# mimbres/neural-audio-fp

Hardware: NVIDIA B200
Metric: search_queries_per_s (higher is better)
Workload: dtype bf16 scan, f32 re-rank

## Files before the change

include/nafp.h:

```cpp
#ifndef NAFP_H_
#define NAFP_H_

#include <stdint.h>

#ifdef __cplusplus
extern "C" {
#endif

typedef struct nafp_ctx nafp_ctx;
typedef struct nafp_index nafp_index;

typedef enum {
    NAFP_OK = 0,
    NAFP_ERR_INVALID = -1,
    NAFP_ERR_CUDA = -2,
    NAFP_ERR_STATE = -3,
    NAFP_ERR_UNSUPPORTED = -4
} nafp_status;

enum { NAFP_INDEX_FLAT_L2 = 0, NAFP_INDEX_IVFPQ = 1, NAFP_INDEX_IVF_FLAT = 2, NAFP_INDEX_IVFPQR = 3 };

int nafp_version(void);
const char* nafp_last_error(void);
int nafp_device_count(void);

int nafp_ctx_create(int device, nafp_ctx** out);
int nafp_ctx_destroy(nafp_ctx* ctx);
int nafp_sync(nafp_ctx* ctx);
void* nafp_ctx_stream(nafp_ctx* ctx);
int nafp_ctx_set_stream(nafp_ctx* ctx, void* cuda_stream);
int64_t nafp_ctx_launch_count(nafp_ctx* ctx);

int nafp_malloc(nafp_ctx* ctx, int64_t bytes, void** out_dev);
int nafp_free(nafp_ctx* ctx, void* dev);
int nafp_malloc_host(nafp_ctx* ctx, int64_t bytes, void** out_host);
int nafp_free_host(nafp_ctx* ctx, void* host);
int nafp_memcpy_h2d(nafp_ctx* ctx, void* dst_dev, const void* src_host, int64_t bytes);
int nafp_memcpy_d2h(nafp_ctx* ctx, void* dst_host, const void* src_dev, int64_t bytes);
int nafp_timer_start(nafp_ctx* ctx);
int nafp_timer_stop(nafp_ctx* ctx, float* out_ms);

int nafp_synth_fp_rows(nafp_ctx* ctx, int64_t seed, int64_t row0, int64_t n_rows, int32_t track_len,
                       float rho, float* out_dev);
int nafp_synth_audio(nafp_ctx* ctx, int64_t seed, int64_t seg0, int64_t n_seg, float* out_dev);


int nafp_weights_load(nafp_ctx* ctx, const float* const* conv_w, const float* const* conv_b,
                      const float* const* ln_g, const float* const* ln_b, const float* div_w1,
                      const float* div_b1, const float* div_w2, const float* div_b2);

int nafp_logmel_forward(nafp_ctx* ctx, const float* x_dev, int64_t n_seg, int64_t group_size,
                        float* mel_dev);

int nafp_logmel_forward_raw(nafp_ctx* ctx, const float* x_dev, int64_t n_seg, int64_t group_size,
                            float* mel_dev, int32_t* group_max_dev);

int nafp_logmel_set_segment_norm(nafp_ctx* ctx, int32_t enable);

int nafp_encoder_forward(nafp_ctx* ctx, const float* mel_dev, int64_t n_seg, float* emb_dev);

int nafp_fingerprint(nafp_ctx* ctx, const float* x_dev, int64_t n_seg, int64_t group_size,
                     float* emb_dev);
int nafp_fingerprint_host(nafp_ctx* ctx, const float* x_host, int64_t n_seg, int64_t group_size,
                          float* emb_host);
int nafp_fingerprint_pcm16_host(nafp_ctx* ctx, const int16_t* pcm_host, int64_t n_seg,
                                int64_t group_size, float* emb_host);
int nafp_fingerprint_pcm16_tracks_host(nafp_ctx* ctx, const int16_t* pcm_host, int64_t n_samples,
                                       const int64_t* seg_off_host, const int32_t* seg_valid_host,
                                       int64_t n_seg, int64_t group_size, float* emb_host);
int nafp_encoder_activation_host(nafp_ctx* ctx, int layer, int64_t n_seg, float* out_host);

int nafp_index_create(nafp_ctx* ctx, int type, int d, int nlist, int pq_m, int pq_nbits,
                      nafp_index** out);
int nafp_index_destroy(nafp_index* idx);
int nafp_index_train(nafp_index* idx, const float* x_host, int64_t n, int64_t seed);
int nafp_index_add(nafp_index* idx, const float* x_host, int64_t n);
int nafp_index_add_dev(nafp_index* idx, const float* x_dev, int64_t n);
int nafp_index_ivfpq_get_params(nafp_index* idx, float* coarse_host, float* pq_host);
int nafp_index_ivfpq_set_params(nafp_index* idx, const float* coarse_host, const float* pq_host);
int nafp_index_ivfpqr_get_refine(nafp_index* idx, float* refine_pq_host);
int nafp_index_ivfpqr_set_refine(nafp_index* idx, const float* refine_pq_host);
int nafp_index_ivf_get_coarse(nafp_index* idx, float* coarse_host);
int nafp_index_ivf_set_coarse(nafp_index* idx, const float* coarse_host);
int nafp_index_reserve(nafp_index* idx, int64_t n_total);
int64_t nafp_index_ntotal(nafp_index* idx);
int nafp_index_is_trained(nafp_index* idx);
int nafp_index_set_nprobe(nafp_index* idx, int nprobe);
int nafp_index_set_label_offset(nafp_index* idx, int64_t offset);
int nafp_index_set_search_rows(nafp_index* idx, int64_t n_rows);

int nafp_index_search(nafp_index* idx, const float* q_host, int64_t nq, int k, float* D_host,
                      int64_t* I_host);
int nafp_index_search_dev(nafp_index* idx, const float* q_dev, int64_t nq, int k, float* D_dev,
                          int64_t* I_dev);
int nafp_index_reconstruct_host(nafp_index* idx, int64_t i0, int64_t n, float* out_host);
int nafp_index_last_search_stats(nafp_index* idx, int64_t* out8);

int nafp_index_profile_scans(nafp_index* idx, int enable, double* total_ms, int64_t* n_scans);

int nafp_index_debug_last_pass(nafp_index* idx, int32_t* flags256, float* thr256, int32_t* total256);
int nafp_index_debug_enable(nafp_index* idx, int32_t* cnt_out, int32_t* first_out, int32_t* grid_out);

int nafp_seq_match(nafp_index* idx, const float* q_host, int64_t n_query_rows,
                   const int64_t* test_ids, int64_t n_test, const int32_t* seq_lens, int32_t n_len,
                   int32_t k_probe, int64_t* pred_ids_host, float* pred_scores_host);

int nafp_seq_plan_dev(nafp_ctx* ctx, const int64_t* test_ids_dev, int64_t n_test, int32_t max_len,
                      int64_t n_query_rows, int32_t* scratch_dev, int32_t* rowmap_dev,
                      int32_t* uniq_rows_dev, int64_t* n_uniq_out);
int nafp_seq_gather_rows_dev(nafp_ctx* ctx, const float* q_dev, const int32_t* rows_dev, int64_t n_rows,
                             float* out_dev);
int nafp_seq_cand_dev(nafp_index* idx, const float* q_dev, int64_t n_query_rows,
                      const int64_t* test_ids_dev, int64_t n_test, const int32_t* seq_lens_dev,
                      int32_t n_len, int32_t max_len, int32_t k_probe, const int64_t* I_dev,
                      const int32_t* rowmap_dev, int64_t n_rows_global, int64_t owned_lo, int64_t owned_hi,
                      int64_t* cand_ids_dev, float* cand_scores_dev, int32_t* n_cand_dev);
int nafp_seq_top_dev(nafp_ctx* ctx, int64_t n_test, int32_t n_len, const int64_t* cand_ids_dev,
                     const float* cand_scores_dev, const int32_t* n_cand_dev,
                     int64_t* pred_ids_dev, float* pred_scores_dev);
int nafp_topk_merge_dev(nafp_ctx* ctx, const float* D_all_dev, const int64_t* I_all_dev,
                        int32_t n_shards, int64_t nq, int32_t k, float* D_out_dev, int64_t* I_out_dev);

int nafp_pairwise_dists_host(nafp_ctx* ctx, const float* q_host, const float* db_host, int64_t n_q, int64_t n_aug,
                             int64_t n_db, int64_t d, int32_t return_dotprod, int32_t squared, float* out_host);
int nafp_conv_eye_host(nafp_ctx* ctx, const float* x_host, int64_t n_aug, int64_t n_q, int64_t n_db, int32_t s,
                       float* out_host);
int nafp_mini_search_host(nafp_ctx* ctx, const float* q_host, const float* db_host, int64_t n_q, int64_t n_aug,
                          int64_t n_db, int64_t d, const int32_t* scopes, int32_t n_scopes, int32_t argmax,
                          int64_t gt_id_offset, double* top1, double* top3, double* top10, double* mean_rank);

#ifdef __cplusplus
}
#endif
#endif
```

neural-audio-fp_b200/csrc/flat_search.cu:

```cuda
#include <cfloat>
#include <climits>
#include <cstdlib>
#include <cstring>
#include <vector>

#include "index.h"
#include "ptx.cuh"

namespace nafp {

__global__ void flat_convert_rows_kernel(const float* __restrict__ x32, __nv_bfloat16* __restrict__ x16,
                                         float* __restrict__ hn, int32_t* __restrict__ maxn2, int64_t row0,
                                         int64_t n) {
    const int lane = threadIdx.x & 31;
    const int64_t warp = (static_cast<int64_t>(blockIdx.x) * blockDim.x + threadIdx.x) >> 5;
    const int64_t nwarps = (static_cast<int64_t>(gridDim.x) * blockDim.x) >> 5;
    float mx = 0.f;
    for (int64_t r = row0 + warp; r < row0 + n; r += nwarps) {
        const float4 v = reinterpret_cast<const float4*>(x32 + r * D128)[lane];
        __nv_bfloat162 a = __floats2bfloat162_rn(v.x, v.y);
        __nv_bfloat162 b = __floats2bfloat162_rn(v.z, v.w);
        uint2 packed;
        packed.x = *reinterpret_cast<uint32_t*>(&a);
        packed.y = *reinterpret_cast<uint32_t*>(&b);
        reinterpret_cast<uint2*>(x16 + r * D128)[lane] = packed;
        float ss = v.x * v.x + v.y * v.y + v.z * v.z + v.w * v.w;
#pragma unroll
        for (int o = 16; o > 0; o >>= 1) ss += __shfl_xor_sync(0xffffffffu, ss, o);
        if (lane == 0) hn[r] = 0.5f * ss;
        mx = fmaxf(mx, ss);
    }
    if (lane == 0 && mx > 0.f) atomicMax(maxn2, __float_as_int(mx));
}

__global__ void flat_fill_kernel(float* hn, int64_t from, int64_t to, float v) {
    int64_t i = from + static_cast<int64_t>(blockIdx.x) * blockDim.x + threadIdx.x;
    if (i < to) hn[i] = v;
}

__global__ void flat_prep_kernel(const float* __restrict__ q_all, const int32_t* __restrict__ src_list, int src_off,
                                 int64_t p0, int nq, int nq_pad, int grid_scan,
                                 __nv_bfloat16* __restrict__ qbf, float* __restrict__ q32,
                                 float* __restrict__ qn2, int32_t* __restrict__ Mx, int32_t* __restrict__ Tg,
                                 int32_t* __restrict__ flags, int64_t* __restrict__ gidx, int32_t* __restrict__ tile_counter) {
    const int lane = threadIdx.x & 31;
    const int row = (blockIdx.x * blockDim.x + threadIdx.x) >> 5;
    if (blockIdx.x == 0 && threadIdx.x == 0) *tile_counter = 0;
    if (row >= nq_pad) return;
    int64_t g = -1;
    if (row < nq) g = src_list ? static_cast<int64_t>(src_list[src_off + row]) : p0 + row;
    float4 v = make_float4(0.f, 0.f, 0.f, 0.f);
    if (g >= 0) v = reinterpret_cast<const float4*>(q_all + g * D128)[lane];
    __nv_bfloat162 a = __floats2bfloat162_rn(v.x, v.y);
    __nv_bfloat162 b = __floats2bfloat162_rn(v.z, v.w);
    uint2 packed;
    packed.x = *reinterpret_cast<uint32_t*>(&a);
    packed.y = *reinterpret_cast<uint32_t*>(&b);
    reinterpret_cast<uint2*>(qbf + row * D128)[lane] = packed;
    reinterpret_cast<float4*>(q32 + row * D128)[lane] = v;
    float ss = v.x * v.x + v.y * v.y + v.z * v.z + v.w * v.w;
#pragma unroll
    for (int o = 16; o > 0; o >>= 1) ss += __shfl_xor_sync(0xffffffffu, ss, o);
    if (lane == 0) {
        qn2[row] = ss;
        Tg[row] = INT_MIN;
        flags[row] = 0;
        gidx[row] = g;
    }
    for (int c = lane; c < grid_scan; c += 32) Mx[row * grid_scan + c] = INT_MIN;
}

constexpr int RING_SLOTS = 4;
constexpr int EPI_WARPS = 16;
constexpr int SCAN_THREADS = (3 + EPI_WARPS) * 32;
constexpr int TMA_WARP = EPI_WARPS + 1, MMA_WARP = EPI_WARPS + 2;
constexpr int EPI_PARTS = EPI_WARPS / 4;
constexpr int PART_COLS = SCAN_TILE / EPI_PARTS;
constexpr int SLOT_BYTES = SCAN_TILE * 128;
constexpr int BOX_BYTES = TILE_ROWS * 128;
constexpr int Q_KB_BYTES = NQ_MAX * 128;
constexpr int Q_BYTES_MAX = 2 * Q_KB_BYTES;
constexpr int H_RING = 4;
constexpr int WARM_TILES = 8;
constexpr int SCAN_SMEM = Q_BYTES_MAX + RING_SLOTS * SLOT_BYTES + H_RING * SCAN_TILE * 4 + 2 * NQ_MAX * 4 + 256 + 1024;
constexpr int NEG_INF_ORD = static_cast<int>(0x807FFFFFu);
static_assert(PART_COLS == 64, "epilogue reads two 32-column chunks per unit");

struct ScanBars {
    uint64_t full[RING_SLOTS];
    uint64_t empty[RING_SLOTS];
    uint64_t tfull[2];
    uint64_t tempty[2];
    uint64_t qfull;
    uint32_t tmem_base;
    int done;
    int tile_of[8];
};

__device__ __forceinline__ void smem_red_max(int* p, int v) {
    asm volatile("red.shared.max.s32 [%0], %1;" ::"r"(smem_u32(p)), "r"(v) : "memory");
}
__device__ __forceinline__ int smem_atom_inc(int* p) {
    int old;
    asm volatile("atom.shared.add.u32 %0, [%1], 1;" : "=r"(old) : "r"(smem_u32(p)) : "memory");
    return old;
}
__device__ __forceinline__ int smem_atom_add(int* p, int v) {
    int old;
    asm volatile("atom.shared.add.u32 %0, [%1], %2;" : "=r"(old) : "r"(smem_u32(p)), "r"(v) : "memory");
    return old;
}
__device__ __forceinline__ int smem_ld_volatile(const int* p) {
    int v;
    asm volatile("ld.volatile.shared.s32 %0, [%1];" : "=r"(v) : "r"(smem_u32(p)) : "memory");
    return v;
}
__device__ __forceinline__ float fmax3(float a, float b, float c) {
    float d;
    asm("max.f32 %0, %1, %2, %3;" : "=f"(d) : "f"(a), "f"(b), "f"(c));
    return d;
}
__device__ __forceinline__ void mbar_arrive_lane0(uint64_t* bar, int lane) {
    asm volatile(
        "{\n\t.reg .pred p;\n\tsetp.eq.s32 p, %1, 0;\n\t@p mbarrier.arrive.shared::cta.b64 _, [%0];\n\t}" ::"r"(smem_u32(bar)),
        "r"(lane)
        : "memory");
}
template <bool EDGE>
__device__ __forceinline__ void scan_chunk_hits(const uint32_t (&v)[32], const float* __restrict__ hc, float t_exact, int nvalid,
                                                uint32_t rbase, int* cnt_q, int* lmax_q, uint64_t* pool_q) {
    uint32_t m = 0;
    float best = -INFINITY;
#pragma unroll
    for (int j = 0; j < 32; ++j) {
        if (!EDGE || j < nvalid) {
            const float sj = __uint_as_float(v[j]) - hc[j];
            m |= (sj > t_exact) ? (1u << j) : 0u;
            best = fmaxf(best, sj);
        }
    }
    if (m) {
        smem_red_max(lmax_q, f2ord(best));
        int pos = smem_atom_add(cnt_q, __popc(m));
        while (m) {
            const int j = __ffs(m) - 1;
            m &= m - 1;
            if (pos < POOL_CAP) pool_q[pos] = rbase + j;
            ++pos;
        }
    }
}

__global__ void __launch_bounds__(SCAN_THREADS, 1)
flat_scan_kernel(const __grid_constant__ CUtensorMap tmap_q, const __grid_constant__ CUtensorMap tmap_db,
                 const float* __restrict__ hn, int32_t* __restrict__ tile_counter, int64_t n_search, int n_tiles, int nq,
                 int n_half, int kg, int32_t* __restrict__ Mx, int32_t* __restrict__ Tg, uint64_t* __restrict__ pool,
                 int32_t* __restrict__ cnt, int32_t* __restrict__ flags, int32_t* __restrict__ dbg_first, int tune) {
    extern __shared__ uint8_t smem_raw[];
    uint8_t* smem = reinterpret_cast<uint8_t*>((reinterpret_cast<uintptr_t>(smem_raw) + 1023) & ~uintptr_t(1023));
    uint8_t* q_s = smem;
    uint8_t* b_s = smem + Q_BYTES_MAX;
    float* h_s = reinterpret_cast<float*>(b_s + RING_SLOTS * SLOT_BYTES);
    int* lmax_s = reinterpret_cast<int*>(h_s + H_RING * SCAN_TILE);
    int* cnt_s = lmax_s + NQ_MAX;
    ScanBars* bars = reinterpret_cast<ScanBars*>(cnt_s + NQ_MAX);

    const int warp = threadIdx.x >> 5;
    const int lane = threadIdx.x & 31;
    const int G = gridDim.x;
    const int cta = blockIdx.x;
    const int warm_cap = ((tune >> 8) & 15) ? ((tune >> 8) & 15) : WARM_TILES;
    const int warm = (tune & 2) ? 1 : max(1, min(warm_cap, n_tiles / G));

    for (int i = threadIdx.x; i < NQ_MAX; i += blockDim.x) {
        lmax_s[i] = INT_MIN;
        cnt_s[i] = 0;
    }
    if (threadIdx.x == 0) {
        tma_prefetch_desc(&tmap_q);
        tma_prefetch_desc(&tmap_db);
        for (int s = 0; s < RING_SLOTS; ++s) {
            mbar_init(&bars->full[s], 1);
            mbar_init(&bars->empty[s], 1);
        }
        for (int a = 0; a < 2; ++a) {
            mbar_init(&bars->tfull[a], 1);
            mbar_init(&bars->tempty[a], EPI_WARPS);
        }
        mbar_init(&bars->qfull, 1);
        bars->done = 0;
        mbar_fence_init();
    }
    if (warp == MMA_WARP) {
        tmem_alloc(&bars->tmem_base, 512);
        tmem_relinquish();
    }
    tc_fence_before();
    __syncthreads();
    tc_fence_after();
    const uint32_t tmem_base = __shfl_sync(0xffffffffu, bars->tmem_base, 0);

    if (warp == TMA_WARP) {
        if (lane == 0) {
            const int q_rows = n_half * 128;
            mbar_arrive_expect_tx(&bars->qfull, 2u * q_rows * 128u);
            for (int kb = 0; kb < 2; ++kb)
                for (int r0 = 0; r0 < q_rows; r0 += 32)
                    tma_load_2d(q_s + kb * Q_KB_BYTES + r0 * 128, &tmap_q, &bars->qfull, kb * 64, r0);
            int tile = cta;
            int revisit = -1;
            int nxt = warm * G + atomicAdd(tile_counter, 1);
            for (int i = 0;; ++i) {
                const int kc0 = 2 * i;
                const uint32_t ph = (kc0 / RING_SLOTS) & 1;
                const int s0 = kc0 % RING_SLOTS;
                mbar_wait_parked(&bars->empty[s0], ph ^ 1);
                bars->tile_of[i & 7] = tile;
                if (tile < 0) {
                    mbar_arrive(&bars->full[s0]);
                    break;
                }
#pragma unroll
                for (int kb = 0; kb < 2; ++kb) {
                    const int s = s0 + kb;
                    if (kb == 1) mbar_wait_parked(&bars->empty[s], ph ^ 1);
                    mbar_arrive_expect_tx(&bars->full[s], SLOT_BYTES + (kb == 0 ? SCAN_TILE * 4 : 0));
                    if (kb == 0)
                        bulk_load_1d(h_s + (i % H_RING) * SCAN_TILE, hn + static_cast<int64_t>(tile) * SCAN_TILE, SCAN_TILE * 4,
                                     &bars->full[s]);
                    uint8_t* dst = b_s + s * SLOT_BYTES;
                    tma_load_2d(dst, &tmap_db, &bars->full[s], kb * 64, tile * SCAN_TILE);
                    tma_load_2d(dst + BOX_BYTES, &tmap_db, &bars->full[s], kb * 64, tile * SCAN_TILE + TILE_ROWS);
                }
                if (i + 1 < warm) {
                    tile = cta + (i + 1) * G;
                } else if (revisit < 0 && nxt < n_tiles) {
                    tile = nxt;
                    nxt = warm * G + atomicAdd(tile_counter, 1);
                } else {
                    ++revisit;
                    tile = revisit < warm ? cta + revisit * G : -1;
                }
            }
        }
        __syncwarp();
    } else if (warp == MMA_WARP) {
        const bool leader = elect_one();
        const uint32_t idesc = umma_idesc_f16(1u, 128u, static_cast<uint32_t>(SCAN_TILE));
        const uint64_t adesc0 = umma_desc_sw128(smem_u32(q_s));
        const uint64_t bdesc0 = umma_desc_sw128(smem_u32(b_s));
        mbar_wait_parked(&bars->qfull, 0);
        uint32_t uc = 0;
        bool more = true;
        for (int i = 0; more; ++i) {
            const int s0 = (2 * i) % RING_SLOTS, s1 = s0 + 1;
            const uint32_t ph = ((2 * i) / RING_SLOTS) & 1;
            for (int hq = 0; hq < n_half; ++hq, ++uc) {
                const int acc = uc & 1;
                const uint32_t aph = (uc >> 1) & 1;
                const bool last = hq == n_half - 1;
                mbar_wait_parked(&bars->tempty[acc], aph ^ 1);
                if (hq == 0) {
                    mbar_wait_parked(&bars->full[s0], ph);
                    if (smem_ld_volatile(&bars->tile_of[i & 7]) < 0) {
                        if (leader) tc_commit(&bars->tfull[acc]);
                        __syncwarp();
                        more = false;
                        break;
                    }
                }
                tc_fence_after();
                const uint32_t d_tmem = tmem_base + acc * SCAN_TILE;
                const uint64_t a_kb0 = adesc0 + static_cast<uint64_t>((hq * (128 * 128)) >> 4);
                const uint64_t a_kb1 = a_kb0 + static_cast<uint64_t>(Q_KB_BYTES >> 4);
                const uint64_t b_kb0 = bdesc0 + static_cast<uint64_t>((s0 * SLOT_BYTES) >> 4);
                const uint64_t b_kb1 = b_kb0 + static_cast<uint64_t>(SLOT_BYTES >> 4);
                if (leader) {
#pragma unroll
                    for (int j = 0; j < 4; ++j) tc_mma_f16(d_tmem, a_kb0 + 2 * j, b_kb0 + 2 * j, idesc, j != 0 ? 1u : 0u);
                    if (last) tc_commit(&bars->empty[s0]);
                }
                if (hq == 0) {
                    mbar_wait_parked(&bars->full[s1], ph);
                    tc_fence_after();
                }
                if (leader) {
#pragma unroll
                    for (int j = 0; j < 4; ++j) tc_mma_f16(d_tmem, a_kb1 + 2 * j, b_kb1 + 2 * j, idesc, 1u);
                    if (last) tc_commit(&bars->empty[s1]);
                    tc_commit(&bars->tfull[acc]);
                }
                __syncwarp();
            }
        }
        __syncwarp();
    } else if (warp < EPI_WARPS) {
        const int qd = warp & 3;
        const int e = warp;
        const int part = e >> 2;
        constexpr int QPW = NQ_MAX / EPI_WARPS;
        const float NEG_INF = -INFINITY;
        int pub = INT_MIN;
        int thr_ord[2] = {NEG_INF_ORD, NEG_INF_ORD};
        float t_exact[2], t_pre[2];
        bool active[2];
#pragma unroll
        for (int hq = 0; hq < 2; ++hq) {
            active[hq] = hq < n_half && (hq * 128 + qd * 32 + lane) < nq;
            t_exact[hq] = active[hq] ? NEG_INF : INFINITY;
            t_pre[hq] = t_exact[hq];
        }
        uint64_t* my_pool = pool + static_cast<int64_t>(cta) * NQ_MAX * POOL_CAP;
        const uint32_t ns32 = static_cast<uint32_t>(n_search);
        auto load_thresholds = [&](int (&tg)[2]) {
#pragma unroll
            for (int hq = 0; hq < 2; ++hq) tg[hq] = active[hq] ? ld_relaxed(&Tg[hq * 128 + qd * 32 + lane]) : INT_MIN;
        };
        auto apply_thresholds = [&](const int (&tg)[2], int i) -> bool {
            bool valid = true;
#pragma unroll
            for (int hq = 0; hq < 2; ++hq) {
                if (active[hq]) {
                    if (tg[hq] > thr_ord[hq]) {
                        if (dbg_first && part == 0 && thr_ord[hq] == NEG_INF_ORD)
                            dbg_first[cta * NQ_MAX + hq * 128 + qd * 32 + lane] = i;
                        thr_ord[hq] = tg[hq];
                        const float t = ord2f(tg[hq]);
                        t_exact[hq] = t;
                        t_pre[hq] = t - fabsf(t) * (1.f / 1048576.f) - 1e-37f;
                    }
                    valid = valid && (thr_ord[hq] > NEG_INF_ORD);
                }
            }
            return __all_sync(0xffffffffu, valid);
        };
        auto publish_maxima = [&]() {
            const int q = e * QPW + lane;
            if (lane < QPW && q < nq) {
                const int m = smem_ld_volatile(&lmax_s[q]);
                if (m > pub) {
                    st_relaxed(&Mx[q * G + cta], m);
                    pub = m;
                }
            }
        };
        const bool probe = dbg_first != nullptr && threadIdx.x == 0 && nq <= 248;
        unsigned long long t_start = 0;
        if (probe) asm volatile("mov.u64 %0, %%globaltimer;" : "=l"(t_start));
        auto stamp = [&](int slot) {
            if (probe) {
                unsigned long long t;
                asm volatile("mov.u64 %0, %%globaltimer;" : "=l"(t));
                dbg_first[cta * NQ_MAX + 248 + slot] = static_cast<int>(t - t_start);
            }
        };
        const uint32_t tlane = tmem_base + (static_cast<uint32_t>(qd * 32) << 16) + part * PART_COLS;
        uint32_t uc = 0;

        for (int w = 0; w < warm; ++w) {
            const uint32_t row0 = static_cast<uint32_t>(cta + w * G) * SCAN_TILE + part * PART_COLS;
            const float* h_part = h_s + (w % H_RING) * SCAN_TILE + part * PART_COLS;
            bool edge = (static_cast<uint32_t>(cta + w * G) + 1u) * SCAN_TILE > ns32 || (tune & 4);
            float hx = 0.f;
            for (int hq = 0; hq < n_half; ++hq, ++uc) {
                const int acc = uc & 1;
                mbar_wait_parked(&bars->tfull[acc], (uc >> 1) & 1);
                if (hq == 0 && !edge) {
                    const float a = h_part[lane], b = h_part[32 + lane];
                    const float hmax_w = __uint_as_float(__reduce_max_sync(0xffffffffu, __float_as_uint(fmaxf(a, b))));
                    const float hmin_w = __uint_as_float(__reduce_min_sync(0xffffffffu, __float_as_uint(fminf(a, b))));
                    hx = hmax_w * (1.f + 1.f / 1048576.f);
                    edge = !(hmax_w - hmin_w <= hmax_w * (1.f / 262144.f));
                }
                tc_fence_after();
                float munit = NEG_INF;
#pragma unroll 1
                for (int c = 0; c < PART_COLS / 32; ++c) {
                    uint32_t v[32];
                    tmem_ld_32x32(tlane + acc * SCAN_TILE + c * 32, v);
                    tc_wait_ld();
                    if (!edge) {
                        float gm[4];
#pragma unroll
                        for (int g = 0; g < 4; ++g) {
                            float m = fmax3(__uint_as_float(v[8 * g]), __uint_as_float(v[8 * g + 1]), __uint_as_float(v[8 * g + 2]));
                            m = fmax3(m, __uint_as_float(v[8 * g + 3]), __uint_as_float(v[8 * g + 4]));
                            m = fmax3(m, __uint_as_float(v[8 * g + 5]), __uint_as_float(v[8 * g + 6]));
                            gm[g] = fmaxf(m, __uint_as_float(v[8 * g + 7]));
                        }
                        munit = fmaxf(munit, fmaxf(fmax3(gm[0], gm[1], gm[2]), gm[3]) - hx);
                    } else {
                        const float* hc = h_part + c * 32;
                        const int nvalid = static_cast<int>(min(ns32 - min(ns32, row0 + c * 32), 32u));
#pragma unroll
                        for (int j = 0; j < 32; ++j)
                            if (j < nvalid) munit = fmaxf(munit, __uint_as_float(v[j]) - hc[j]);
                    }
                }
                if (hq == 0 ? active[0] : active[1]) smem_red_max(&lmax_s[hq * 128 + qd * 32 + lane], f2ord(munit));
                tc_fence_before();
                __syncwarp();
                mbar_arrive_lane0(&bars->tempty[acc], lane);
            }
            publish_maxima();
            if (w == 0) stamp(0);
        }
        {
            int tg[2];
            bool ok = false;
            for (int spin = 0; spin < 4096 && !ok; ++spin) {
                publish_maxima();
                load_thresholds(tg);
                ok = apply_thresholds(tg, 1);
                if (!ok) __nanosleep(100);
            }
            stamp(1);
        }
        for (int i = warm;; ++i) {
            int tg[2] = {INT_MIN, INT_MIN};
            const bool rf = i > warm && (((tune & 8) && i < warm + 32) || (i & 3) == 0);
            if (rf) load_thresholds(tg);
            const float* h_part = h_s + (i % H_RING) * SCAN_TILE + part * PART_COLS;
            uint32_t row0 = 0;
            float hm = 0.f;
            bool end = false, edge = false;
            for (int hq = 0; hq < n_half; ++hq, ++uc) {
                const int acc = uc & 1;
                mbar_wait_parked(&bars->tfull[acc], (uc >> 1) & 1);
                if (hq == 0) {
                    const int tile = smem_ld_volatile(&bars->tile_of[i & 7]);
                    if (tile < 0) {
                        end = true;
                        break;
                    }
                    row0 = static_cast<uint32_t>(tile) * SCAN_TILE + part * PART_COLS;
                    const float hmin_w =
                        __uint_as_float(__reduce_min_sync(0xffffffffu, __float_as_uint(fminf(h_part[lane], h_part[32 + lane]))));
                    hm = hmin_w * (1.f - 1.f / 1048576.f);
                    edge = (static_cast<uint32_t>(tile) + 1u) * SCAN_TILE > ns32 || (tune & 4);
                }
                const float tp = (hq == 0 ? t_pre[0] : t_pre[1]) + hm;
                tc_fence_after();
                const uint32_t taddr = tlane + acc * SCAN_TILE;
#pragma unroll 1
                for (int c = 0; c < PART_COLS / 32; ++c) {
                    uint32_t v[32];
                    tmem_ld_32x32(taddr + c * 32, v);
                    tc_wait_ld();
                    float gm[4];
#pragma unroll
                    for (int g = 0; g < 4; ++g) {
                        float m = fmax3(__uint_as_float(v[8 * g]), __uint_as_float(v[8 * g + 1]), __uint_as_float(v[8 * g + 2]));
                        m = fmax3(m, __uint_as_float(v[8 * g + 3]), __uint_as_float(v[8 * g + 4]));
                        m = fmax3(m, __uint_as_float(v[8 * g + 5]), __uint_as_float(v[8 * g + 6]));
                        gm[g] = fmaxf(m, __uint_as_float(v[8 * g + 7]));
                    }
                    const float ma = fmaxf(fmax3(gm[0], gm[1], gm[2]), gm[3]);
                    const bool fired = ma > tp;
                    if (__any_sync(0xffffffffu, fired)) {
                        const int q = hq * 128 + qd * 32 + lane;
                        const float te = hq == 0 ? t_exact[0] : t_exact[1];
                        const uint32_t rbase = row0 + c * 32;
                        if (!edge)
                            scan_chunk_hits<false>(v, h_part + c * 32, te, 32, rbase, &cnt_s[q], &lmax_s[q], my_pool + q * POOL_CAP);
                        else
                            scan_chunk_hits<true>(v, h_part + c * 32, te, static_cast<int>(min(ns32 - min(ns32, rbase), 32u)), rbase,
                                                  &cnt_s[q], &lmax_s[q], my_pool + q * POOL_CAP);
                        __syncwarp();
                    }
                }
                tc_fence_before();
                __syncwarp();
                mbar_arrive_lane0(&bars->tempty[acc], lane);
            }
            if (end) break;
            if (rf) apply_thresholds(tg, i);
            if (i < warm + 32 || (i & 3) == 0) publish_maxima();
            if (i == warm) stamp(2);
            if (i == 16) stamp(5);
            if (i == 32) stamp(6);
            if (i == 96) stamp(7);
        }
        stamp(3);
        publish_maxima();
        stamp(4);
        __syncwarp();
        asm volatile("bar.sync 1, %0;" ::"n"(EPI_WARPS * 32) : "memory");
        {
            const int q = e * QPW + lane;
            if (lane < QPW && q < nq) {
                const int c = cnt_s[q];
                cnt[cta * NQ_MAX + q] = min(c, POOL_CAP);
                if (c > POOL_CAP) flags[q] = 1;
            }
        }
        if (lane == 0) smem_atom_inc(&bars->done);
    } else {
        uint32_t round = 0;
        while (smem_ld_volatile(&bars->done) < EPI_WARPS) {
            for (int q = cta; q < nq; q += G) {
                uint32_t u[5];
#pragma unroll
                for (int t = 0; t < 5; ++t) {
                    const int g = lane + 32 * t;
                    const int m = g < G ? ld_relaxed(&Mx[q * G + g]) : INT_MIN;
                    u[t] = static_cast<uint32_t>(m) ^ 0x80000000u;
                }
                uint32_t res = 0;
                for (int bit = 31; bit >= 0; --bit) {
                    const uint32_t cand = res | (1u << bit);
                    int c = 0;
#pragma unroll
                    for (int t = 0; t < 5; ++t) c += (u[t] >= cand) ? 1 : 0;
                    c = __reduce_add_sync(0xffffffffu, c);
                    if (c >= kg) res = cand;
                }
                const int T = static_cast<int>(res ^ 0x80000000u);
                if (lane == 0 && T > NEG_INF_ORD && T > ld_relaxed(&Tg[q])) st_relaxed(&Tg[q], T);
            }
            ++round;
            if ((tune & 1) || round < 6) {
                __nanosleep((tune & 1) ? (round < 48 ? 100 : (round < 96 ? 1000 : 4000)) : 100);
            } else {
                for (int nap = 0; nap < 8 && smem_ld_volatile(&bars->done) < EPI_WARPS; ++nap) __nanosleep(500);
            }
        }
    }

    tc_fence_before();
    __syncthreads();
    if (warp == MMA_WARP) tmem_dealloc(tmem_base, 512);
}

__device__ __forceinline__ uint64_t score_key(float s, uint32_t row) {
    return (static_cast<uint64_t>(static_cast<uint32_t>(f2ord(s)) ^ 0x80000000u) << 32) | (0xFFFFFFFFu - row);
}
__device__ __forceinline__ float key_score(uint64_t key) {
    return ord2f(static_cast<int>(static_cast<uint32_t>(key >> 32) ^ 0x80000000u));
}
__device__ __forceinline__ uint32_t key_row(uint64_t key) { return 0xFFFFFFFFu - static_cast<uint32_t>(key); }

__device__ void bitonic_sort_desc(uint64_t* keys, int n) {
    for (int k = 2; k <= n; k <<= 1) {
        for (int j = k >> 1; j > 0; j >>= 1) {
            for (int i = threadIdx.x; i < n; i += blockDim.x) {
                const int ixj = i ^ j;
                if (ixj > i) {
                    const uint64_t a = keys[i], b = keys[ixj];
                    const bool desc = (i & k) == 0;
                    if (desc ? (a < b) : (a > b)) {
                        keys[i] = b;
                        keys[ixj] = a;
                    }
                }
            }
            __syncthreads();
        }
    }
}

struct SelBatch {
    int np[SEL_SLOTS];
    int grid_alloc;
};

__global__ void __launch_bounds__(256)
flat_select_kernel(SelBatch batch, int k, int grid_scan, int64_t n_rows, const float* __restrict__ q32,
                   const float* __restrict__ qn2, const float* __restrict__ x32, const float* __restrict__ hn,
                   const int32_t* __restrict__ maxn2, const int32_t* __restrict__ Tg,
                   const uint64_t* __restrict__ pool, const int32_t* __restrict__ cnt, int32_t* __restrict__ flags,
                   const int64_t* __restrict__ gidx, int32_t* __restrict__ fail_list, int32_t* __restrict__ fail_count,
                   int64_t label_offset, float* __restrict__ D, int64_t* __restrict__ I,
                   unsigned long long* __restrict__ stats) {
    __shared__ uint64_t keys[SELECT_CAP];
    __shared__ int total_s;
    const int q = blockIdx.x;
    const int slot = blockIdx.y;
    if (q >= batch.np[slot]) return;
    q32 += static_cast<int64_t>(slot) * NQ_MAX * D128;
    qn2 += slot * NQ_MAX;
    Tg += slot * NQ_MAX;
    pool += static_cast<int64_t>(slot) * batch.grid_alloc * NQ_MAX * POOL_CAP;
    cnt += static_cast<int64_t>(slot) * batch.grid_alloc * NQ_MAX;
    flags += slot * NQ_MAX;
    gidx += slot * NQ_MAX;
    const int64_t g = gidx[q];
    if (flags[q] != 0) {
        if (threadIdx.x == 0) {
            fail_list[atomicAdd(fail_count, 1)] = static_cast<int32_t>(g);
            atomicAdd(&stats[5], 1ull);
        }
        return;
    }
    if (threadIdx.x == 0) total_s = 0;
    __syncthreads();
    bool over = false;
    for (int g = threadIdx.x; g < grid_scan; g += blockDim.x) {
        const int c = cnt[g * NQ_MAX + q];
        if (c > 0) {
            const int base = atomicAdd(&total_s, c);
            if (base + c <= SELECT_CAP) {
                const uint64_t* src = pool + (static_cast<int64_t>(g) * NQ_MAX + q) * POOL_CAP;
                for (int i = 0; i < c; ++i) keys[base + i] = src[i];
            } else {
                over = true;
            }
        }
    }
    if (__syncthreads_or(over ? 1 : 0)) {
        if (threadIdx.x == 0) {
            flags[q] = 1;
            fail_list[atomicAdd(fail_count, 1)] = static_cast<int32_t>(g);
            atomicAdd(&stats[5], 1ull);
        }
        return;
    }
    const int total = total_s;
    const int64_t need = n_rows < k ? n_rows : k;
    if (total < need) {
        if (threadIdx.x == 0) {
            flags[q] = 1;
            fail_list[atomicAdd(fail_count, 1)] = static_cast<int32_t>(g);
            atomicAdd(&stats[5], 1ull);
        }
        return;
    }
    const int warp = threadIdx.x >> 5, lane = threadIdx.x & 31;
    const int sub = lane >> 3, l8 = lane & 7;
    float4 qv[4];
#pragma unroll
    for (int c = 0; c < 4; ++c) qv[c] = reinterpret_cast<const float4*>(q32 + q * D128 + l8 * 16)[c];
    for (int i0 = warp * 4; i0 < total; i0 += 32) {
        const int i = i0 + sub;
        const bool ok = i < total;
        const uint32_t row = ok ? static_cast<uint32_t>(keys[i]) : 0u;
        const float4* xr = reinterpret_cast<const float4*>(x32 + static_cast<int64_t>(row) * D128 + l8 * 16);
        const float4 a0 = xr[0], a1 = xr[1], a2 = xr[2], a3 = xr[3];
        const float hh = hn[row];
        float s = a0.x * qv[0].x + a0.y * qv[0].y + a0.z * qv[0].z + a0.w * qv[0].w;
        s += a1.x * qv[1].x + a1.y * qv[1].y + a1.z * qv[1].z + a1.w * qv[1].w;
        s += a2.x * qv[2].x + a2.y * qv[2].y + a2.z * qv[2].z + a2.w * qv[2].w;
        s += a3.x * qv[3].x + a3.y * qv[3].y + a3.z * qv[3].z + a3.w * qv[3].w;
        s += __shfl_xor_sync(0xffffffffu, s, 4);
        s += __shfl_xor_sync(0xffffffffu, s, 2);
        s += __shfl_xor_sync(0xffffffffu, s, 1);
        __syncwarp();
        if (ok && l8 == 0) keys[i] = score_key(s - hh, row);
    }
    int npow = 1;
    while (npow < total) npow <<= 1;
    __syncthreads();
    for (int i = total + threadIdx.x; i < npow; i += blockDim.x) keys[i] = 0;
    __syncthreads();
    bitonic_sort_desc(keys, npow);
    const int tgo = Tg[q];
    if (tgo > NEG_INF_ORD) {
        const float qn = sqrtf(qn2[q]);
        const float xn = sqrtf(__int_as_float(*maxn2));
        const float u = 0.00390625f;
        const float eps = (2.f * u + u * u) * qn * xn * 1.01f + 1e-5f * qn * xn + 1e-30f;
        const float bound = ord2f(tgo) + eps;
        const float sk = key_score(keys[need - 1]);
        if (!(sk > bound)) {
            if (threadIdx.x == 0) {
                flags[q] = 2;
                fail_list[atomicAdd(fail_count, 1)] = static_cast<int32_t>(g);
                atomicAdd(&stats[6], 1ull);
            }
            return;
        }
    }
    for (int j = threadIdx.x; j < k; j += blockDim.x) {
        if (j < need) {
            const uint64_t key = keys[j];
            D[g * k + j] = fmaxf(qn2[q] - 2.f * key_score(key), 0.f);
            I[g * k + j] = static_cast<int64_t>(key_row(key)) + label_offset;
        } else {
            D[g * k + j] = INFINITY;
            I[g * k + j] = -1;
        }
    }
    if (threadIdx.x == 0) atomicAdd(&stats[3], static_cast<unsigned long long>(total));
}

__global__ void __launch_bounds__(256)
flat_brute_scan_kernel(int k, int64_t n_rows, const float* __restrict__ q_all, const float* __restrict__ x32,
                       const float* __restrict__ hn, const int32_t* __restrict__ list, int64_t list_off,
                       uint64_t* __restrict__ part) {
    __shared__ uint64_t lists[8][MAX_K];
    const int e = blockIdx.y;
    const int64_t g = list ? static_cast<int64_t>(list[list_off + e]) : list_off + e;
    const int chunk = blockIdx.x;
    const int warp = threadIdx.x >> 5, lane = threadIdx.x & 31;
    const int64_t per = (n_rows + BRUTE_CHUNKS - 1) / BRUTE_CHUNKS;
    const int64_t r0 = chunk * per;
    const int64_t r1 = r0 + per < n_rows ? r0 + per : n_rows;
    uint64_t* lst = lists[warp];
    for (int i = lane; i < k; i += 32) lst[i] = 0;
    __syncwarp();
    const float4 qv = reinterpret_cast<const float4*>(q_all + g * D128)[lane];
    uint64_t kth = 0;
    for (int64_t r = r0 + warp; r < r1; r += 8) {
        const float s = warp_dot128(qv, x32 + r * D128, lane) - hn[r];
        const uint64_t key = score_key(s, static_cast<uint32_t>(r));
        if (key > kth) {
            if (lane == 0) {
                int p = k - 1;
                while (p > 0 && lst[p - 1] < key) {
                    lst[p] = lst[p - 1];
                    --p;
                }
                lst[p] = key;
            }
            __syncwarp();
            kth = lst[k - 1];
            __syncwarp();
        }
    }
    __syncthreads();
    if (warp == 0) {
        uint64_t* out = part + (static_cast<int64_t>(e) * BRUTE_CHUNKS + chunk) * MAX_K;
        int head = 0;
        for (int j = 0; j < k; ++j) {
            uint64_t cand = (lane < 8 && head < k) ? lists[lane][head] : 0;
            uint64_t best = cand;
#pragma unroll
            for (int o = 16; o > 0; o >>= 1) {
                const uint64_t other = __shfl_xor_sync(0xffffffffu, best, o);
                best = other > best ? other : best;
            }
            if (lane < 8 && cand == best && best != 0) ++head;
            if (lane == 0) out[j] = best;
        }
    }
}

__global__ void __launch_bounds__(256)
flat_brute_merge_kernel(int k, const float* __restrict__ q_all, const int32_t* __restrict__ list, int64_t list_off,
                        uint64_t* __restrict__ part, int64_t label_offset, float* __restrict__ D,
                        int64_t* __restrict__ I, unsigned long long* __restrict__ stats) {
    __shared__ uint64_t red[8];
    __shared__ uint64_t winner;
    __shared__ float qn2_s;
    const int e = blockIdx.x;
    const int64_t g = list ? static_cast<int64_t>(list[list_off + e]) : list_off + e;
    uint64_t* p = part + static_cast<int64_t>(e) * BRUTE_CHUNKS * MAX_K;
    const int warp = threadIdx.x >> 5, lane = threadIdx.x & 31;
    if (warp == 0) {
        const float4 v = reinterpret_cast<const float4*>(q_all + g * D128)[lane];
        float ss = v.x * v.x + v.y * v.y + v.z * v.z + v.w * v.w;
#pragma unroll
        for (int o = 16; o > 0; o >>= 1) ss += __shfl_xor_sync(0xffffffffu, ss, o);
        if (lane == 0) qn2_s = ss;
    }
    __syncthreads();
    for (int j = 0; j < k; ++j) {
        uint64_t best = 0;
        for (int c = threadIdx.x; c < BRUTE_CHUNKS * k; c += blockDim.x) {
            const uint64_t v = p[(c / k) * MAX_K + (c % k)];
            best = v > best ? v : best;
        }
#pragma unroll
        for (int o = 16; o > 0; o >>= 1) {
            const uint64_t other = __shfl_xor_sync(0xffffffffu, best, o);
            best = other > best ? other : best;
        }
        if (lane == 0) red[warp] = best;
        __syncthreads();
        if (threadIdx.x == 0) {
            uint64_t b = 0;
            for (int w = 0; w < 8; ++w) b = red[w] > b ? red[w] : b;
            winner = b;
            if (b != 0) {
                D[g * k + j] = fmaxf(qn2_s - 2.f * key_score(b), 0.f);
                I[g * k + j] = static_cast<int64_t>(key_row(b)) + label_offset;
            } else {
                D[g * k + j] = INFINITY;
                I[g * k + j] = -1;
            }
        }
        __syncthreads();
        const uint64_t w = winner;
        if (w != 0)
            for (int c = threadIdx.x; c < BRUTE_CHUNKS * k; c += blockDim.x) {
                uint64_t* slot = &p[(c / k) * MAX_K + (c % k)];
                if (*slot == w) *slot = 0;
            }
        __syncthreads();
    }
    if (threadIdx.x == 0) atomicAdd(&stats[1], 1ull);
}

constexpr int PROF_RING = 8192;
static int64_t round_up(int64_t v, int64_t m) { return (v + m - 1) / m * m; }

int index_reserve(nafp_index* idx, int64_t n_total) {
    if (n_total <= idx->cap) return NAFP_OK;
    nafp_ctx* ctx = idx->ctx;
    const int64_t new_cap = round_up(n_total, TILE_ROWS);
    float* x32 = nullptr;
    __nv_bfloat16* x16 = nullptr;
    float* hn = nullptr;
    NAFP_CUDA(cudaMalloc(&x32, static_cast<size_t>(new_cap) * idx->d * sizeof(float)));
    if (idx->scan_copy) {
        NAFP_CUDA(cudaMalloc(&x16, static_cast<size_t>(new_cap) * idx->d * sizeof(__nv_bfloat16)));
        NAFP_CUDA(cudaMalloc(&hn, static_cast<size_t>(new_cap + SCAN_TILE) * sizeof(float)));
        NAFP_CUDA(cudaMemsetAsync(x16, 0, static_cast<size_t>(new_cap) * idx->d * sizeof(__nv_bfloat16), ctx->stream));
    }
    if (idx->n > 0) {
        NAFP_CUDA(cudaMemcpyAsync(x32, idx->x32, static_cast<size_t>(idx->n) * idx->d * sizeof(float),
                                  cudaMemcpyDeviceToDevice, ctx->stream));
        if (idx->scan_copy) {
            NAFP_CUDA(cudaMemcpyAsync(x16, idx->x16, static_cast<size_t>(idx->n) * idx->d * sizeof(__nv_bfloat16),
                                      cudaMemcpyDeviceToDevice, ctx->stream));
            NAFP_CUDA(cudaMemcpyAsync(hn, idx->hn, static_cast<size_t>(idx->n) * sizeof(float),
                                      cudaMemcpyDeviceToDevice, ctx->stream));
        }
    }
    if (idx->scan_copy) {
        const int64_t cnt = new_cap + SCAN_TILE - idx->n;
        const int threads = 256;
        const int64_t blocks = (cnt + threads - 1) / threads;
        flat_fill_kernel<<<static_cast<unsigned>(blocks), threads, 0, ctx->stream>>>(hn, idx->n, new_cap + SCAN_TILE, INFINITY);
        ctx->launches++;
        NAFP_CUDA(cudaGetLastError());
    }
    NAFP_CUDA(cudaStreamSynchronize(ctx->stream));
    if (idx->x32) cudaFree(idx->x32);
    if (idx->x16) cudaFree(idx->x16);
    if (idx->hn) cudaFree(idx->hn);
    idx->x32 = x32;
    idx->x16 = x16;
    idx->hn = hn;
    idx->cap = new_cap;
    if (!idx->scan_copy) return NAFP_OK;
    const uint64_t dims[2] = {static_cast<uint64_t>(idx->d), static_cast<uint64_t>(new_cap)};
    const uint64_t strides[2] = {2, static_cast<uint64_t>(idx->d) * 2};
    const uint32_t box[2] = {64, TILE_ROWS};
    NAFP_TRY(make_tensor_map(&idx->tmap_db, CU_TENSOR_MAP_DATA_TYPE_BFLOAT16, 2, x16, dims, strides, box, nullptr,
                             CU_TENSOR_MAP_SWIZZLE_128B));
    idx->tmap_db_valid = true;
    return NAFP_OK;
}

int flat_add_dev(nafp_index* idx, const float* x, int64_t n, bool src_is_host) {
    if (n == 0) return NAFP_OK;
    nafp_ctx* ctx = idx->ctx;
    NAFP_CUDA(cudaSetDevice(ctx->device));
    if (idx->n + n > idx->cap) {
        int64_t want = idx->cap * 2;
        if (want < idx->n + n) want = idx->n + n;
        NAFP_TRY(index_reserve(idx, want));
    }
    NAFP_CUDA(cudaMemcpyAsync(idx->x32 + idx->n * idx->d, x, static_cast<size_t>(n) * idx->d * sizeof(float),
                              src_is_host ? cudaMemcpyHostToDevice : cudaMemcpyDeviceToDevice, ctx->stream));
    if (idx->scan_copy) {
        const int threads = 256;
        int64_t blocks = (n * 32 + threads - 1) / threads;
        if (blocks > ctx->sm_count * 16) blocks = ctx->sm_count * 16;
        flat_convert_rows_kernel<<<static_cast<unsigned>(blocks), threads, 0, ctx->stream>>>(idx->x32, idx->x16, idx->hn,
                                                                                            idx->maxn2, idx->n, n);
        ctx->launches++;
        NAFP_CUDA(cudaGetLastError());
    }
    if (src_is_host) NAFP_CUDA(cudaStreamSynchronize(ctx->stream));
    idx->n += n;
    return NAFP_OK;
}

static int ensure_scratch(nafp_index* idx) {
    if (idx->scratch_ready) return NAFP_OK;
    nafp_ctx* ctx = idx->ctx;
    idx->grid = ctx->sm_count;
    NAFP_REQUIRE(idx->grid <= 160, NAFP_ERR_UNSUPPORTED, "flat scan: %d SMs (reducer handles <= 160)", idx->grid);
    const int G = idx->grid;
    NAFP_CUDA(cudaMalloc(&idx->qbf, NQ_MAX * D128 * sizeof(__nv_bfloat16)));
    NAFP_CUDA(cudaMalloc(&idx->q32, SEL_SLOTS * NQ_MAX * D128 * sizeof(float)));
    NAFP_CUDA(cudaMalloc(&idx->qn2, SEL_SLOTS * NQ_MAX * sizeof(float)));
    NAFP_CUDA(cudaMalloc(&idx->Mx, static_cast<size_t>(NQ_MAX) * G * sizeof(int32_t)));
    NAFP_CUDA(cudaMalloc(&idx->Tg, SEL_SLOTS * NQ_MAX * sizeof(int32_t)));
    NAFP_CUDA(cudaMalloc(&idx->pool, SEL_SLOTS * static_cast<size_t>(G) * NQ_MAX * POOL_CAP * sizeof(uint64_t)));
    NAFP_CUDA(cudaMalloc(&idx->cnt, SEL_SLOTS * static_cast<size_t>(G) * NQ_MAX * sizeof(int32_t)));
    NAFP_CUDA(cudaMalloc(&idx->flags, SEL_SLOTS * NQ_MAX * sizeof(int32_t)));
    NAFP_CUDA(cudaMalloc(&idx->gidx, SEL_SLOTS * NQ_MAX * sizeof(int64_t)));
    NAFP_CUDA(cudaMalloc(&idx->brute_part, static_cast<size_t>(BRUTE_SLOTS) * BRUTE_CHUNKS * MAX_K * sizeof(uint64_t)));
    NAFP_CUDA(cudaMalloc(&idx->stats, 8 * sizeof(unsigned long long)));
    NAFP_CUDA(cudaMalloc(&idx->tile_counter, sizeof(int32_t)));
    NAFP_CUDA(cudaMemsetAsync(idx->stats, 0, 8 * sizeof(unsigned long long), ctx->stream));
    const uint64_t dims[2] = {static_cast<uint64_t>(D128), static_cast<uint64_t>(NQ_MAX)};
    const uint64_t strides[2] = {2, static_cast<uint64_t>(D128) * 2};
    const uint32_t box[2] = {64, 32};
    NAFP_TRY(make_tensor_map(&idx->tmap_q, CU_TENSOR_MAP_DATA_TYPE_BFLOAT16, 2, idx->qbf, dims, strides, box, nullptr,
                             CU_TENSOR_MAP_SWIZZLE_128B));
    NAFP_CUDA(cudaFuncSetAttribute(flat_scan_kernel, cudaFuncAttributeMaxDynamicSharedMemorySize, SCAN_SMEM));
    idx->scratch_ready = true;
    return NAFP_OK;
}

static int brute_rounds(nafp_index* idx, const float* q_dev, const int32_t* list, int64_t first, int64_t count, int k,
                        int64_t n_search, float* D_dev, int64_t* I_dev) {
    nafp_ctx* ctx = idx->ctx;
    for (int64_t off = 0; off < count; off += BRUTE_SLOTS) {
        const int n = static_cast<int>(count - off < BRUTE_SLOTS ? count - off : BRUTE_SLOTS);
        flat_brute_scan_kernel<<<dim3(BRUTE_CHUNKS, n), 256, 0, ctx->stream>>>(k, n_search, q_dev, idx->x32, idx->hn, list,
                                                                              first + off, idx->brute_part);
        flat_brute_merge_kernel<<<n, 256, 0, ctx->stream>>>(k, q_dev, list, first + off, idx->brute_part, idx->label_offset,
                                                            D_dev, I_dev, idx->stats);
        ctx->launches += 2;
    }
    NAFP_CUDA(cudaGetLastError());
    return NAFP_OK;
}

static int scan_tune() {
    static const int v = [] { const char* e = getenv("NAFP_SCAN_TUNE"); return e ? atoi(e) : 0; }();
    return v;
}

static int scan_pass(nafp_index* idx, const float* q_dev, const int32_t* src_list, int src_off, int64_t p0, int np, int kg,
                     int grid_scan, int n_tiles, int64_t n_search, int slot) {
    nafp_ctx* ctx = idx->ctx;
    const int n_half = np > 128 ? 2 : 1;
    const int nq_pad = n_half * 128;
    const int64_t G = idx->grid;
    float* q32 = idx->q32 + static_cast<int64_t>(slot) * NQ_MAX * D128;
    float* qn2 = idx->qn2 + slot * NQ_MAX;
    int32_t* Tg = idx->Tg + slot * NQ_MAX;
    uint64_t* pool = idx->pool + static_cast<int64_t>(slot) * G * NQ_MAX * POOL_CAP;
    int32_t* cnt = idx->cnt + static_cast<int64_t>(slot) * G * NQ_MAX;
    int32_t* flags = idx->flags + slot * NQ_MAX;
    int64_t* gidx = idx->gidx + slot * NQ_MAX;
    flat_prep_kernel<<<(nq_pad * 32 + 255) / 256, 256, 0, ctx->stream>>>(q_dev, src_list, src_off, p0, np, nq_pad, grid_scan,
                                                                         idx->qbf, q32, qn2, idx->Mx, Tg, flags, gidx, idx->tile_counter);
    const bool prof = idx->profile && idx->prof_n < PROF_RING;
    if (prof) cudaEventRecord(idx->prof_ev[2 * idx->prof_n], ctx->stream);
    flat_scan_kernel<<<grid_scan, SCAN_THREADS, SCAN_SMEM, ctx->stream>>>(idx->tmap_q, idx->tmap_db, idx->hn, idx->tile_counter, n_search,
                                                                          n_tiles, np, n_half, kg, idx->Mx, Tg, pool, cnt, flags,
                                                                          idx->dbg_first, scan_tune());
    if (prof) {
        cudaEventRecord(idx->prof_ev[2 * idx->prof_n + 1], ctx->stream);
        idx->prof_n++;
    }
    ctx->launches += 2;
    idx->last_slot = slot;
    return NAFP_OK;
}

static int select_batch(nafp_index* idx, const SelBatch& batch, int n_slots, int k, int grid_scan, int64_t n_search,
                        int32_t* fail_list, int32_t* fail_count, float* D_dev, int64_t* I_dev) {
    nafp_ctx* ctx = idx->ctx;
    flat_select_kernel<<<dim3(NQ_MAX, n_slots), 256, 0, ctx->stream>>>(batch, k, grid_scan, n_search, idx->q32, idx->qn2, idx->x32,
                                                                       idx->hn, idx->maxn2, idx->Tg, idx->pool, idx->cnt, idx->flags,
                                                                       idx->gidx, fail_list, fail_count, idx->label_offset, D_dev,
                                                                       I_dev, idx->stats);
    ctx->launches++;
    return NAFP_OK;
}

int flat_search_dev(nafp_index* idx, const float* q_dev, int64_t nq, int k, float* D_dev, int64_t* I_dev) {
    nafp_ctx* ctx = idx->ctx;
    NAFP_REQUIRE(k >= 1 && k <= MAX_K, NAFP_ERR_INVALID, "search: k=%d outside [1,%d]", k, MAX_K);
    NAFP_REQUIRE(idx->d == D128, NAFP_ERR_UNSUPPORTED, "search: d=%d (the tensor-core scan is built for d=128)", idx->d);
    NAFP_REQUIRE(idx->scan_copy, NAFP_ERR_STATE, "search: this index keeps no bf16 scan copy of its rows (IVF-PQ types)");
    NAFP_REQUIRE(nq < (1ll << 31), NAFP_ERR_INVALID, "search: more than 2^31 query rows in one call");
    NAFP_CUDA(cudaSetDevice(ctx->device));
    NAFP_TRY(ensure_scratch(idx));
    if (nq == 0) return NAFP_OK;
    const int64_t n_search = (idx->search_rows >= 0 && idx->search_rows < idx->n) ? idx->search_rows : idx->n;
    const int n_tiles = static_cast<int>((n_search + SCAN_TILE - 1) / SCAN_TILE);
    const int kg = k + 28;
    const int grid_scan = n_tiles < idx->grid ? (n_tiles > 0 ? n_tiles : 1) : idx->grid;
    const bool brute = (n_search < 8192) || (kg > grid_scan) || (k > 64);
    idx->host_rows += nq;
    if (brute) return brute_rounds(idx, q_dev, nullptr, 0, nq, k, n_search, D_dev, I_dev);

    if (idx->fail_cap < 2 * nq) {
        if (idx->fail_list) cudaFree(idx->fail_list);
        idx->fail_list = nullptr;
        idx->fail_cap = 0;
        NAFP_CUDA(cudaMalloc(&idx->fail_list, static_cast<size_t>(2 * nq + 2) * sizeof(int32_t)));
        idx->fail_cap = 2 * nq;
    }
    int32_t* list1 = idx->fail_list;
    int32_t* list2 = idx->fail_list + nq;
    int32_t* counts = idx->fail_list + 2 * nq;
    NAFP_CUDA(cudaMemsetAsync(counts, 0, 2 * sizeof(int32_t), ctx->stream));
    SelBatch batch;
    batch.grid_alloc = idx->grid;
    int slot = 0;
    for (int64_t p0 = 0; p0 < nq; p0 += NQ_MAX) {
        const int np = static_cast<int>(nq - p0 < NQ_MAX ? nq - p0 : NQ_MAX);
        NAFP_TRY(scan_pass(idx, q_dev, nullptr, 0, p0, np, kg, grid_scan, n_tiles, n_search, slot));
        batch.np[slot++] = np;
        idx->host_passes++;
        if (slot == SEL_SLOTS || p0 + NQ_MAX >= nq) {
            NAFP_TRY(select_batch(idx, batch, slot, k, grid_scan, n_search, list1, counts, D_dev, I_dev));
            slot = 0;
        }
    }
    NAFP_CUDA(cudaGetLastError());
    int32_t h[2] = {0, 0};
    NAFP_CUDA(cudaMemcpyAsync(h, counts, sizeof(h), cudaMemcpyDeviceToHost, ctx->stream));
    NAFP_CUDA(cudaStreamSynchronize(ctx->stream));
    if (h[0] > 0) {
        const int kg_retry = 2 * kg < grid_scan - 2 ? 2 * kg : (grid_scan - 2 > kg ? grid_scan - 2 : kg);
        slot = 0;
        for (int off = 0; off < h[0]; off += NQ_MAX) {
            const int np = h[0] - off < NQ_MAX ? h[0] - off : NQ_MAX;
            NAFP_TRY(scan_pass(idx, q_dev, list1, off, 0, np, kg_retry, grid_scan, n_tiles, n_search, slot));
            batch.np[slot++] = np;
            idx->host_passes++;
            if (slot == SEL_SLOTS || off + NQ_MAX >= h[0]) {
                NAFP_TRY(select_batch(idx, batch, slot, k, grid_scan, n_search, list2, counts + 1, D_dev, I_dev));
                slot = 0;
            }
        }
        NAFP_CUDA(cudaMemcpyAsync(h, counts, sizeof(h), cudaMemcpyDeviceToHost, ctx->stream));
        NAFP_CUDA(cudaStreamSynchronize(ctx->stream));
        if (h[1] > 0) NAFP_TRY(brute_rounds(idx, q_dev, list2, 0, h[1], k, n_search, D_dev, I_dev));
    }
    NAFP_CUDA(cudaGetLastError());
    return NAFP_OK;
}

}

using namespace nafp;

extern "C" {

int nafp_index_create(nafp_ctx* ctx, int type, int d, int nlist, int pq_m, int pq_nbits, nafp_index** out) {
    NAFP_REQUIRE(ctx && out, NAFP_ERR_INVALID, "nafp_index_create: NULL argument");
    *out = nullptr;
    NAFP_REQUIRE(type == NAFP_INDEX_FLAT_L2 || type == NAFP_INDEX_IVFPQ || type == NAFP_INDEX_IVF_FLAT || type == NAFP_INDEX_IVFPQR,
                 NAFP_ERR_UNSUPPORTED, "nafp_index_create: index type %d is not built (l2, ivfpq, ivf, ivfpq-rr)", type);
    NAFP_REQUIRE(d == D128, NAFP_ERR_UNSUPPORTED, "nafp_index_create: d=%d; only d=128 (MODEL.EMB_SZ) is built", d);
    NAFP_CUDA(cudaSetDevice(ctx->device));
    nafp_index* idx = new nafp_index();
    idx->ctx = ctx;
    idx->type = type;
    idx->d = d;
    idx->scan_copy = type == NAFP_INDEX_FLAT_L2 || type == NAFP_INDEX_IVF_FLAT;
    if (cudaMalloc(&idx->maxn2, sizeof(int32_t)) != cudaSuccess ||
        cudaMemsetAsync(idx->maxn2, 0, sizeof(int32_t), ctx->stream) != cudaSuccess) {
        set_error("nafp_index_create: cudaMalloc failed");
        delete idx;
        return NAFP_ERR_CUDA;
    }
    if (type != NAFP_INDEX_FLAT_L2) {
        int s = type == NAFP_INDEX_IVF_FLAT ? ivfflat_create(idx, nlist) : ivfpq_create(idx, nlist, pq_m, pq_nbits);
        if (s == NAFP_OK && type == NAFP_INDEX_IVFPQR) s = ivfpqr_enable(idx);
        if (s != NAFP_OK) {
            if (idx->ivf) ivfpq_destroy(idx);
            cudaFree(idx->maxn2);
            delete idx;
            return s;
        }
    }
    *out = idx;
    return NAFP_OK;
}

int nafp_index_destroy(nafp_index* idx) {
    if (!idx) return NAFP_OK;
    cudaSetDevice(idx->ctx->device);
    cudaStreamSynchronize(idx->ctx->stream);
    if (idx->ivf) ivfpq_destroy(idx);
    for (auto& e : idx->prof_ev) cudaEventDestroy(e);
    void* bufs[] = {idx->x32, idx->x16, idx->hn, idx->tile_counter, idx->maxn2, idx->qbf, idx->q32, idx->qn2, idx->Mx, idx->Tg,
                    idx->pool, idx->cnt, idx->flags, idx->gidx, idx->fail_list, idx->brute_part, idx->stats, idx->dbg_first, idx->stage_q, idx->stage_D,
                    idx->stage_I};
    for (void* b : bufs)
        if (b) cudaFree(b);
    delete idx;
    return NAFP_OK;
}

int nafp_index_train(nafp_index* idx, const float* x_host, int64_t n, int64_t seed) {
    NAFP_RANGE("nafp_index_train");
    NAFP_REQUIRE(idx, NAFP_ERR_INVALID, "nafp_index_train: idx is NULL");
    if (idx->type == NAFP_INDEX_FLAT_L2) return NAFP_OK;
    NAFP_REQUIRE(x_host && n > 0, NAFP_ERR_INVALID, "nafp_index_train: empty training set");
    return ivfpq_train(idx, x_host, n, seed);
}

int nafp_index_is_trained(nafp_index* idx);

static int add_common(nafp_index* idx, const float* x, int64_t n, bool host) {
    NAFP_REQUIRE(idx && (n == 0 || x) && n >= 0, NAFP_ERR_INVALID, "nafp_index_add: bad arguments");
    NAFP_REQUIRE(idx->n + n < (1ll << 32), NAFP_ERR_UNSUPPORTED, "nafp_index_add: more than 2^32 rows per shard");
    if (idx->type != NAFP_INDEX_FLAT_L2)
        NAFP_REQUIRE(nafp_index_is_trained(idx) == 1, NAFP_ERR_STATE, "nafp_index_add: IVF index is not trained");
    const int64_t row0 = idx->n;
    NAFP_TRY(flat_add_dev(idx, x, n, host));
    if (idx->type != NAFP_INDEX_FLAT_L2) NAFP_TRY(ivfpq_add_rows(idx, row0, n));
    return NAFP_OK;
}
int nafp_index_add(nafp_index* idx, const float* x_host, int64_t n) {
    NAFP_RANGE("nafp_index_add");
    return add_common(idx, x_host, n, true);
}
int nafp_index_add_dev(nafp_index* idx, const float* x_dev, int64_t n) {
    NAFP_RANGE("nafp_index_add_dev");
    return add_common(idx, x_dev, n, false);
}

int nafp_index_reserve(nafp_index* idx, int64_t n_total) {
    NAFP_REQUIRE(idx && n_total >= 0, NAFP_ERR_INVALID, "nafp_index_reserve: bad arguments");
    NAFP_CUDA(cudaSetDevice(idx->ctx->device));
    return index_reserve(idx, n_total);
}

int64_t nafp_index_ntotal(nafp_index* idx) { return idx ? idx->n : 0; }

int nafp_index_set_nprobe(nafp_index* idx, int nprobe) {
    NAFP_REQUIRE(idx && nprobe >= 1, NAFP_ERR_INVALID, "nafp_index_set_nprobe: bad arguments");
    idx->nprobe = nprobe;
    return NAFP_OK;
}
int nafp_index_set_search_rows(nafp_index* idx, int64_t n_rows) {
    NAFP_REQUIRE(idx, NAFP_ERR_INVALID, "nafp_index_set_search_rows: idx is NULL");
    idx->search_rows = n_rows;
    return NAFP_OK;
}
int nafp_index_set_label_offset(nafp_index* idx, int64_t offset) {
    NAFP_REQUIRE(idx, NAFP_ERR_INVALID, "nafp_index_set_label_offset: idx is NULL");
    idx->label_offset = offset;
    return NAFP_OK;
}

int nafp_index_search_dev(nafp_index* idx, const float* q_dev, int64_t nq, int k, float* D_dev, int64_t* I_dev) {
    NAFP_RANGE("nafp_index_search_dev");
    NAFP_REQUIRE(idx && nq >= 0 && (nq == 0 || (q_dev && D_dev && I_dev)), NAFP_ERR_INVALID,
                 "nafp_index_search_dev: bad arguments");
    if (idx->type != NAFP_INDEX_FLAT_L2) return ivfpq_search_dev(idx, q_dev, nq, k, D_dev, I_dev);
    return flat_search_dev(idx, q_dev, nq, k, D_dev, I_dev);
}

int nafp_index_search(nafp_index* idx, const float* q_host, int64_t nq, int k, float* D_host, int64_t* I_host) {
    NAFP_RANGE("nafp_index_search");
    NAFP_REQUIRE(idx && nq >= 0 && (nq == 0 || (q_host && D_host && I_host)), NAFP_ERR_INVALID,
                 "nafp_index_search: bad arguments");
    NAFP_REQUIRE(k >= 1 && k <= MAX_K, NAFP_ERR_INVALID, "search: k=%d outside [1,%d]", k, MAX_K);
    if (nq == 0) return NAFP_OK;
    nafp_ctx* ctx = idx->ctx;
    NAFP_CUDA(cudaSetDevice(ctx->device));
    if (idx->stage_q_rows < nq) {
        if (idx->stage_q) cudaFree(idx->stage_q);
        idx->stage_q = nullptr;
        idx->stage_q_rows = 0;
        NAFP_CUDA(cudaMalloc(&idx->stage_q, static_cast<size_t>(nq) * idx->d * sizeof(float)));
        idx->stage_q_rows = nq;
    }
    if (idx->stage_out_elems < nq * k) {
        if (idx->stage_D) cudaFree(idx->stage_D);
        if (idx->stage_I) cudaFree(idx->stage_I);
        idx->stage_D = nullptr;
        idx->stage_I = nullptr;
        idx->stage_out_elems = 0;
        NAFP_CUDA(cudaMalloc(&idx->stage_D, static_cast<size_t>(nq) * k * sizeof(float)));
        NAFP_CUDA(cudaMalloc(&idx->stage_I, static_cast<size_t>(nq) * k * sizeof(int64_t)));
        idx->stage_out_elems = nq * k;
    }
    NAFP_CUDA(cudaMemcpyAsync(idx->stage_q, q_host, static_cast<size_t>(nq) * idx->d * sizeof(float),
                              cudaMemcpyHostToDevice, ctx->stream));
    NAFP_TRY(nafp_index_search_dev(idx, idx->stage_q, nq, k, idx->stage_D, idx->stage_I));
    NAFP_CUDA(cudaMemcpyAsync(D_host, idx->stage_D, static_cast<size_t>(nq) * k * sizeof(float), cudaMemcpyDeviceToHost,
                              ctx->stream));
    NAFP_CUDA(cudaMemcpyAsync(I_host, idx->stage_I, static_cast<size_t>(nq) * k * sizeof(int64_t),
                              cudaMemcpyDeviceToHost, ctx->stream));
    NAFP_CUDA(cudaStreamSynchronize(ctx->stream));
    return NAFP_OK;
}

int nafp_index_reconstruct_host(nafp_index* idx, int64_t i0, int64_t n, float* out_host) {
    NAFP_RANGE("nafp_index_reconstruct_host");
    NAFP_REQUIRE(idx && out_host && i0 >= 0 && n >= 0 && i0 + n <= idx->n, NAFP_ERR_INVALID,
                 "nafp_index_reconstruct_host: range [%lld, %lld) outside [0, %lld)", (long long)i0,
                 (long long)(i0 + n), (long long)(idx ? idx->n : 0));
    if (n == 0) return NAFP_OK;
    NAFP_CUDA(cudaMemcpyAsync(out_host, idx->x32 + i0 * idx->d, static_cast<size_t>(n) * idx->d * sizeof(float),
                              cudaMemcpyDeviceToHost, idx->ctx->stream));
    NAFP_CUDA(cudaStreamSynchronize(idx->ctx->stream));
    return NAFP_OK;
}

int nafp_index_debug_enable(nafp_index* idx, int32_t* cnt_out, int32_t* first_out, int32_t* grid_out) {
    NAFP_REQUIRE(idx && idx->scratch_ready, NAFP_ERR_STATE, "debug: search once first");
    nafp_ctx* ctx = idx->ctx;
    NAFP_CUDA(cudaStreamSynchronize(ctx->stream));
    const size_t n = static_cast<size_t>(idx->grid) * NQ_MAX;
    if (!idx->dbg_first) {
        NAFP_CUDA(cudaMalloc(&idx->dbg_first, n * 4));
        NAFP_CUDA(cudaMemset(idx->dbg_first, 0xFF, n * 4));
    }
    if (grid_out) *grid_out = idx->grid;
    if (cnt_out) NAFP_CUDA(cudaMemcpy(cnt_out, idx->cnt + static_cast<size_t>(idx->last_slot) * n, n * 4, cudaMemcpyDeviceToHost));
    if (first_out) {
        NAFP_CUDA(cudaMemcpy(first_out, idx->dbg_first, n * 4, cudaMemcpyDeviceToHost));
        NAFP_CUDA(cudaMemset(idx->dbg_first, 0xFF, n * 4));
    }
    return NAFP_OK;
}

int nafp_index_debug_last_pass(nafp_index* idx, int32_t* flags256, float* thr256, int32_t* total256) {
    NAFP_REQUIRE(idx && idx->scratch_ready && flags256 && thr256 && total256, NAFP_ERR_INVALID, "debug: bad arguments");
    nafp_ctx* ctx = idx->ctx;
    NAFP_CUDA(cudaStreamSynchronize(ctx->stream));
    std::vector<int32_t> tg(NQ_MAX), cnt(static_cast<size_t>(idx->grid) * NQ_MAX);
    NAFP_CUDA(cudaMemcpy(flags256, idx->flags + idx->last_slot * NQ_MAX, NQ_MAX * 4, cudaMemcpyDeviceToHost));
    NAFP_CUDA(cudaMemcpy(tg.data(), idx->Tg + idx->last_slot * NQ_MAX, NQ_MAX * 4, cudaMemcpyDeviceToHost));
    NAFP_CUDA(cudaMemcpy(cnt.data(), idx->cnt + static_cast<size_t>(idx->last_slot) * cnt.size(), cnt.size() * 4, cudaMemcpyDeviceToHost));
    for (int q = 0; q < NQ_MAX; ++q) {
        int32_t o = tg[q];
        uint32_t b = static_cast<uint32_t>(o >= 0 ? o : (o ^ 0x7FFFFFFF));
        memcpy(&thr256[q], &b, 4);
        int64_t t = 0;
        for (int g = 0; g < idx->grid; ++g) t += cnt[static_cast<size_t>(g) * NQ_MAX + q];
        total256[q] = static_cast<int32_t>(t);
    }
    return NAFP_OK;
}

int nafp_index_profile_scans(nafp_index* idx, int enable, double* total_ms, int64_t* n_scans) {
    NAFP_REQUIRE(idx, NAFP_ERR_INVALID, "nafp_index_profile_scans: idx is NULL");
    nafp_ctx* ctx = idx->ctx;
    NAFP_CUDA(cudaStreamSynchronize(ctx->stream));
    double sum = 0.0;
    for (int64_t i = 0; i < idx->prof_n; ++i) {
        float ms = 0.f;
        NAFP_CUDA(cudaEventElapsedTime(&ms, idx->prof_ev[2 * i], idx->prof_ev[2 * i + 1]));
        sum += ms;
    }
    if (total_ms) *total_ms = sum;
    if (n_scans) *n_scans = idx->prof_n;
    idx->prof_n = 0;
    if (enable && idx->prof_ev.empty()) {
        idx->prof_ev.resize(2 * PROF_RING);
        for (auto& e : idx->prof_ev) NAFP_CUDA(cudaEventCreate(&e));
    }
    idx->profile = enable != 0;
    return NAFP_OK;
}

int nafp_index_last_search_stats(nafp_index* idx, int64_t* out4) {
    NAFP_REQUIRE(idx && out4, NAFP_ERR_INVALID, "nafp_index_last_search_stats: bad arguments");
    for (int i = 0; i < 8; ++i) out4[i] = 0;
    if (idx->ivf && idx->type != NAFP_INDEX_IVF_FLAT) {
        ivfpq_take_stats(idx, out4);
        return NAFP_OK;
    }
    if (!idx->stats) return NAFP_OK;
    unsigned long long h[8];
    NAFP_CUDA(cudaMemcpyAsync(h, idx->stats, sizeof(h), cudaMemcpyDeviceToHost, idx->ctx->stream));
    NAFP_CUDA(cudaMemsetAsync(idx->stats, 0, sizeof(h), idx->ctx->stream));
    NAFP_CUDA(cudaStreamSynchronize(idx->ctx->stream));
    for (int i = 0; i < 8; ++i) out4[i] = static_cast<int64_t>(h[i]);
    out4[0] = idx->host_rows;
    out4[2] = idx->host_passes;
    idx->host_rows = idx->host_passes = 0;
    return NAFP_OK;
}

}
```

neural-audio-fp_b200/csrc/index.h:

```cpp
#pragma once
#include <cuda_bf16.h>

#include "common.h"
#include <vector>

namespace nafp {

constexpr int D128 = 128;
constexpr int NQ_MAX = 256;
constexpr int TILE_ROWS = 128;
constexpr int SCAN_TILE = 256;
constexpr int POOL_CAP = 128;
constexpr int MAX_K = 128;
constexpr int BRUTE_CHUNKS = 296;
constexpr int BRUTE_SLOTS = 32;
constexpr int SELECT_CAP = 4096;
constexpr int SEL_SLOTS = 16;

struct IvfPq;

}

struct nafp_index {
    nafp_ctx* ctx = nullptr;
    int type = 0;
    int d = 0;
    int64_t n = 0;
    int64_t cap = 0;
    float* x32 = nullptr;
    __nv_bfloat16* x16 = nullptr;
    float* hn = nullptr;
    int32_t* maxn2 = nullptr;
    bool scan_copy = true;
    int64_t label_offset = 0;
    int64_t search_rows = -1;
    CUtensorMap tmap_db;
    CUtensorMap tmap_q;
    bool tmap_db_valid = false;

    int last_slot = 0;
    bool scratch_ready = false;
    int grid = 0;
    __nv_bfloat16* qbf = nullptr;
    float* q32 = nullptr;
    float* qn2 = nullptr;
    int32_t* Mx = nullptr;
    int32_t* Tg = nullptr;
    uint64_t* pool = nullptr;
    int32_t* cnt = nullptr;
    int32_t* flags = nullptr;
    int64_t* gidx = nullptr;
    int32_t* fail_list = nullptr;
    int64_t fail_cap = 0;
    uint64_t* brute_part = nullptr;
    unsigned long long* stats = nullptr;
    int32_t* tile_counter = nullptr;
    int32_t* dbg_first = nullptr;
    float* stage_q = nullptr;  int64_t stage_q_rows = 0;
    float* stage_D = nullptr;  int64_t* stage_I = nullptr;  int64_t stage_out_elems = 0;

    int64_t host_rows = 0, host_passes = 0;

    bool profile = false;
    std::vector<cudaEvent_t> prof_ev;
    int64_t prof_n = 0;

    int nprobe = 1;
    nafp::IvfPq* ivf = nullptr;
};

namespace nafp {
int flat_search_dev(nafp_index* idx, const float* q_dev, int64_t nq, int k, float* D_dev, int64_t* I_dev);
int flat_add_dev(nafp_index* idx, const float* x_dev, int64_t n, bool src_is_host);
int index_reserve(nafp_index* idx, int64_t n_total);
int ivfpq_create(nafp_index* idx, int nlist, int m, int nbits);
int ivfflat_create(nafp_index* idx, int nlist);
int ivfpqr_enable(nafp_index* idx);
void ivfpq_destroy(nafp_index* idx);
int ivfpq_train(nafp_index* idx, const float* x_host, int64_t n, int64_t seed);
int ivfpq_add_rows(nafp_index* idx, int64_t row0, int64_t n);
int ivfpq_search_dev(nafp_index* idx, const float* q_dev, int64_t nq, int k, float* D_dev, int64_t* I_dev);
void ivfpq_take_stats(nafp_index* idx, int64_t* out8);
}
```

neural-audio-fp_b200/csrc/ptx.cuh:

```cuda
#pragma once
#include <cstdint>
#include <cuda_runtime.h>

namespace nafp {

__device__ __forceinline__ uint32_t smem_u32(const void* p) {
    return static_cast<uint32_t>(__cvta_generic_to_shared(p));
}

__device__ __forceinline__ bool elect_one() {
    uint32_t pred = 0;
    asm volatile(
        "{\n\t.reg .pred P;\n\t"
        "elect.sync _|P, 0xffffffff;\n\t"
        "selp.u32 %0, 1, 0, P;\n\t}\n"
        : "=r"(pred));
    return pred != 0;
}

__device__ __forceinline__ void mbar_init(uint64_t* bar, uint32_t count) {
    asm volatile("mbarrier.init.shared::cta.b64 [%0], %1;" ::"r"(smem_u32(bar)), "r"(count) : "memory");
}
__device__ __forceinline__ void mbar_fence_init() {
    asm volatile("fence.mbarrier_init.release.cluster;" ::: "memory");
}
__device__ __forceinline__ void mbar_arrive(uint64_t* bar) {
    asm volatile("mbarrier.arrive.shared::cta.b64 _, [%0];" ::"r"(smem_u32(bar)) : "memory");
}
__device__ __forceinline__ void mbar_arrive_expect_tx(uint64_t* bar, uint32_t bytes) {
    asm volatile("mbarrier.arrive.expect_tx.shared::cta.b64 _, [%0], %1;" ::"r"(smem_u32(bar)), "r"(bytes) : "memory");
}
__device__ __forceinline__ bool mbar_try_wait(uint64_t* bar, uint32_t parity) {
    uint32_t ok;
    asm volatile(
        "{\n\t.reg .pred P;\n\t"
        "mbarrier.try_wait.parity.shared::cta.b64 P, [%1], %2;\n\t"
        "selp.u32 %0, 1, 0, P;\n\t}\n"
        : "=r"(ok)
        : "r"(smem_u32(bar)), "r"(parity)
        : "memory");
    return ok != 0;
}
__device__ __forceinline__ void mbar_wait(uint64_t* bar, uint32_t parity) {
    uint32_t spins = 0;
    while (!mbar_try_wait(bar, parity)) {
        if (++spins > (1u << 26)) __trap();
    }
}
__device__ __forceinline__ void mbar_wait_parked(uint64_t* bar, uint32_t parity) {
    uint32_t spins = 0;
    for (;;) {
        uint32_t ok;
        asm volatile(
            "{\n\t.reg .pred P;\n\t"
            "mbarrier.try_wait.parity.shared::cta.b64 P, [%1], %2, %3;\n\t"
            "selp.u32 %0, 1, 0, P;\n\t}\n"
            : "=r"(ok)
            : "r"(smem_u32(bar)), "r"(parity), "r"(2000u)
            : "memory");
        if (ok) return;
        if (++spins > (1u << 24)) __trap();
    }
}

__device__ __forceinline__ void tma_prefetch_desc(const void* tmap) {
    asm volatile("prefetch.tensormap [%0];" ::"l"(reinterpret_cast<uint64_t>(tmap)) : "memory");
}
__device__ __forceinline__ void tma_load_2d(void* smem_dst, const void* tmap, uint64_t* bar, int32_t c0, int32_t c1) {
    asm volatile(
        "cp.async.bulk.tensor.2d.shared::cluster.global.mbarrier::complete_tx::bytes [%0], [%1, {%3, %4}], [%2];"
        ::"r"(smem_u32(smem_dst)), "l"(reinterpret_cast<uint64_t>(tmap)), "r"(smem_u32(bar)), "r"(c0), "r"(c1)
        : "memory");
}
__device__ __forceinline__ void tma_load_3d(void* smem_dst, const void* tmap, uint64_t* bar, int32_t c0, int32_t c1, int32_t c2) {
    asm volatile(
        "cp.async.bulk.tensor.3d.shared::cluster.global.mbarrier::complete_tx::bytes [%0], [%1, {%3, %4, %5}], [%2];"
        ::"r"(smem_u32(smem_dst)), "l"(reinterpret_cast<uint64_t>(tmap)), "r"(smem_u32(bar)), "r"(c0), "r"(c1), "r"(c2)
        : "memory");
}
__device__ __forceinline__ void tma_load_4d(void* smem_dst, const void* tmap, uint64_t* bar, int32_t c0, int32_t c1, int32_t c2, int32_t c3) {
    asm volatile(
        "cp.async.bulk.tensor.4d.shared::cluster.global.mbarrier::complete_tx::bytes [%0], [%1, {%3, %4, %5, %6}], [%2];"
        ::"r"(smem_u32(smem_dst)), "l"(reinterpret_cast<uint64_t>(tmap)), "r"(smem_u32(bar)), "r"(c0), "r"(c1), "r"(c2), "r"(c3)
        : "memory");
}
__device__ __forceinline__ void tma_load_5d(void* smem_dst, const void* tmap, uint64_t* bar, int32_t c0, int32_t c1, int32_t c2, int32_t c3, int32_t c4) {
    asm volatile(
        "cp.async.bulk.tensor.5d.shared::cluster.global.mbarrier::complete_tx::bytes [%0], [%1, {%3, %4, %5, %6, %7}], [%2];"
        ::"r"(smem_u32(smem_dst)), "l"(reinterpret_cast<uint64_t>(tmap)), "r"(smem_u32(bar)), "r"(c0), "r"(c1), "r"(c2), "r"(c3), "r"(c4)
        : "memory");
}
__device__ __forceinline__ void tma_store_2d(const void* tmap, const void* smem_src, int32_t c0, int32_t c1) {
    asm volatile("cp.async.bulk.tensor.2d.global.shared::cta.bulk_group [%0, {%2, %3}], [%1];"
                 ::"l"(reinterpret_cast<uint64_t>(tmap)), "r"(smem_u32(smem_src)), "r"(c0), "r"(c1) : "memory");
}
__device__ __forceinline__ void tma_store_commit() { asm volatile("cp.async.bulk.commit_group;" ::: "memory"); }
__device__ __forceinline__ void tma_store_wait_read() { asm volatile("cp.async.bulk.wait_group.read 0;" ::: "memory"); }
__device__ __forceinline__ void tma_store_wait_all() { asm volatile("cp.async.bulk.wait_group 0;" ::: "memory"); }

__device__ __forceinline__ void tma_prefetch_2d(const void* tmap, int32_t c0, int32_t c1) {
    asm volatile("cp.async.bulk.prefetch.tensor.2d.L2.global.tile [%0, {%1, %2}];"
                 ::"l"(reinterpret_cast<uint64_t>(tmap)), "r"(c0), "r"(c1) : "memory");
}
__device__ __forceinline__ void tma_prefetch_4d(const void* tmap, int32_t c0, int32_t c1, int32_t c2, int32_t c3) {
    asm volatile("cp.async.bulk.prefetch.tensor.4d.L2.global.tile [%0, {%1, %2, %3, %4}];"
                 ::"l"(reinterpret_cast<uint64_t>(tmap)), "r"(c0), "r"(c1), "r"(c2), "r"(c3) : "memory");
}
__device__ __forceinline__ void tma_prefetch_5d(const void* tmap, int32_t c0, int32_t c1, int32_t c2, int32_t c3, int32_t c4) {
    asm volatile("cp.async.bulk.prefetch.tensor.5d.L2.global.tile [%0, {%1, %2, %3, %4, %5}];"
                 ::"l"(reinterpret_cast<uint64_t>(tmap)), "r"(c0), "r"(c1), "r"(c2), "r"(c3), "r"(c4) : "memory");
}
__device__ __forceinline__ uint64_t pk2(float a, float b) {
    uint64_t r;
    asm("mov.b64 %0, {%1, %2};" : "=l"(r) : "f"(a), "f"(b));
    return r;
}
__device__ __forceinline__ void upk2(uint64_t v, float& a, float& b) { asm("mov.b64 {%0, %1}, %2;" : "=f"(a), "=f"(b) : "l"(v)); }
__device__ __forceinline__ uint64_t fma2(uint64_t a, uint64_t b, uint64_t c) {
    uint64_t r;
    asm("fma.rn.f32x2 %0, %1, %2, %3;" : "=l"(r) : "l"(a), "l"(b), "l"(c));
    return r;
}
__device__ __forceinline__ uint64_t mul2(uint64_t a, uint64_t b) {
    uint64_t r;
    asm("mul.rn.f32x2 %0, %1, %2;" : "=l"(r) : "l"(a), "l"(b));
    return r;
}
__device__ __forceinline__ uint64_t add2(uint64_t a, uint64_t b) {
    uint64_t r;
    asm("add.rn.f32x2 %0, %1, %2;" : "=l"(r) : "l"(a), "l"(b));
    return r;
}

__device__ __forceinline__ void bulk_load_1d(void* smem_dst, const void* gsrc, uint32_t bytes, uint64_t* bar) {
    asm volatile("cp.async.bulk.shared::cluster.global.mbarrier::complete_tx::bytes [%0], [%1], %2, [%3];" ::"r"(smem_u32(smem_dst)),
                 "l"(reinterpret_cast<uint64_t>(gsrc)), "r"(bytes), "r"(smem_u32(bar))
                 : "memory");
}
__device__ __forceinline__ void fence_proxy_async_smem() {
    asm volatile("fence.proxy.async.shared::cta;" ::: "memory");
}

__device__ __forceinline__ void tmem_alloc(uint32_t* smem_result, uint32_t ncols) {
    asm volatile("tcgen05.alloc.cta_group::1.sync.aligned.shared::cta.b32 [%0], %1;" ::"r"(smem_u32(smem_result)), "r"(ncols) : "memory");
}
__device__ __forceinline__ void tmem_relinquish() {
    asm volatile("tcgen05.relinquish_alloc_permit.cta_group::1.sync.aligned;" ::: "memory");
}
__device__ __forceinline__ void tmem_dealloc(uint32_t taddr, uint32_t ncols) {
    asm volatile("tcgen05.dealloc.cta_group::1.sync.aligned.b32 %0, %1;" ::"r"(taddr), "r"(ncols) : "memory");
}
__device__ __forceinline__ void tc_fence_before() { asm volatile("tcgen05.fence::before_thread_sync;" ::: "memory"); }
__device__ __forceinline__ void tc_fence_after() { asm volatile("tcgen05.fence::after_thread_sync;" ::: "memory"); }
__device__ __forceinline__ void tc_wait_ld() { asm volatile("tcgen05.wait::ld.sync.aligned;" ::: "memory"); }

__device__ __forceinline__ void tc_mma_f16(uint32_t tmem_d, uint64_t adesc, uint64_t bdesc, uint32_t idesc, uint32_t accumulate) {
    asm volatile(
        "{\n\t.reg .pred p;\n\t"
        "setp.ne.b32 p, %4, 0;\n\t"
        "tcgen05.mma.cta_group::1.kind::f16 [%0], %1, %2, %3, p;\n\t}\n"
        ::"r"(tmem_d), "l"(adesc), "l"(bdesc), "r"(idesc), "r"(accumulate)
        : "memory");
}
__device__ __forceinline__ void tc_commit(uint64_t* bar) {
    asm volatile("tcgen05.commit.cta_group::1.mbarrier::arrive::one.shared::cluster.b64 [%0];" ::"r"(smem_u32(bar)) : "memory");
}

__device__ __forceinline__ void tmem_ld_32x32(uint32_t taddr, uint32_t (&v)[32]) {
    asm volatile(
        "tcgen05.ld.sync.aligned.32x32b.x32.b32 "
        "{%0, %1, %2, %3, %4, %5, %6, %7, %8, %9, %10, %11, %12, %13, %14, %15, "
        "%16, %17, %18, %19, %20, %21, %22, %23, %24, %25, %26, %27, %28, %29, %30, %31}, [%32];"
        : "=r"(v[0]), "=r"(v[1]), "=r"(v[2]), "=r"(v[3]), "=r"(v[4]), "=r"(v[5]), "=r"(v[6]), "=r"(v[7]),
          "=r"(v[8]), "=r"(v[9]), "=r"(v[10]), "=r"(v[11]), "=r"(v[12]), "=r"(v[13]), "=r"(v[14]), "=r"(v[15]),
          "=r"(v[16]), "=r"(v[17]), "=r"(v[18]), "=r"(v[19]), "=r"(v[20]), "=r"(v[21]), "=r"(v[22]), "=r"(v[23]),
          "=r"(v[24]), "=r"(v[25]), "=r"(v[26]), "=r"(v[27]), "=r"(v[28]), "=r"(v[29]), "=r"(v[30]), "=r"(v[31])
        : "r"(taddr)
        : "memory");
}
__device__ __forceinline__ void tmem_ld_32x64(uint32_t taddr, uint32_t (&v)[64]) {
    asm volatile(
        "tcgen05.ld.sync.aligned.32x32b.x64.b32 "
        "{%0, %1, %2, %3, %4, %5, %6, %7, %8, %9, %10, %11, %12, %13, %14, %15, %16, %17, %18, %19, %20, %21, %22, %23, %24, %25, %26, %27, %28, %29, %30, %31, %32, %33, %34, %35, %36, %37, %38, %39, %40, %41, %42, %43, %44, %45, %46, %47, %48, %49, %50, %51, %52, %53, %54, %55, %56, %57, %58, %59, %60, %61, %62, %63}, [%64];"
        : "=r"(v[0]), "=r"(v[1]), "=r"(v[2]), "=r"(v[3]), "=r"(v[4]), "=r"(v[5]), "=r"(v[6]), "=r"(v[7]), "=r"(v[8]), "=r"(v[9]), "=r"(v[10]), "=r"(v[11]), "=r"(v[12]), "=r"(v[13]), "=r"(v[14]), "=r"(v[15]), "=r"(v[16]), "=r"(v[17]), "=r"(v[18]), "=r"(v[19]), "=r"(v[20]), "=r"(v[21]), "=r"(v[22]), "=r"(v[23]), "=r"(v[24]), "=r"(v[25]), "=r"(v[26]), "=r"(v[27]), "=r"(v[28]), "=r"(v[29]), "=r"(v[30]), "=r"(v[31]), "=r"(v[32]), "=r"(v[33]), "=r"(v[34]), "=r"(v[35]), "=r"(v[36]), "=r"(v[37]), "=r"(v[38]), "=r"(v[39]), "=r"(v[40]), "=r"(v[41]), "=r"(v[42]), "=r"(v[43]), "=r"(v[44]), "=r"(v[45]), "=r"(v[46]), "=r"(v[47]), "=r"(v[48]), "=r"(v[49]), "=r"(v[50]), "=r"(v[51]), "=r"(v[52]), "=r"(v[53]), "=r"(v[54]), "=r"(v[55]), "=r"(v[56]), "=r"(v[57]), "=r"(v[58]), "=r"(v[59]), "=r"(v[60]), "=r"(v[61]), "=r"(v[62]), "=r"(v[63])
        : "r"(taddr)
        : "memory");
}
__device__ __forceinline__ uint32_t tmem_ld_32x1(uint32_t taddr) {
    uint32_t v;
    asm volatile("tcgen05.ld.sync.aligned.32x32b.x1.b32 {%0}, [%1];" : "=r"(v) : "r"(taddr) : "memory");
    return v;
}
__device__ __forceinline__ void tmem_ld_32x16(uint32_t taddr, uint32_t (&v)[16]) {
    asm volatile(
        "tcgen05.ld.sync.aligned.32x32b.x16.b32 "
        "{%0, %1, %2, %3, %4, %5, %6, %7, %8, %9, %10, %11, %12, %13, %14, %15}, [%16];"
        : "=r"(v[0]), "=r"(v[1]), "=r"(v[2]), "=r"(v[3]), "=r"(v[4]), "=r"(v[5]), "=r"(v[6]), "=r"(v[7]),
          "=r"(v[8]), "=r"(v[9]), "=r"(v[10]), "=r"(v[11]), "=r"(v[12]), "=r"(v[13]), "=r"(v[14]), "=r"(v[15])
        : "r"(taddr)
        : "memory");
}

__device__ __forceinline__ void tmem_st_32x16(uint32_t taddr, const uint32_t (&v)[16]) {
    asm volatile(
        "tcgen05.st.sync.aligned.32x32b.x16.b32 [%0], "
        "{%1, %2, %3, %4, %5, %6, %7, %8, %9, %10, %11, %12, %13, %14, %15, %16};"
        ::"r"(taddr), "r"(v[0]), "r"(v[1]), "r"(v[2]), "r"(v[3]), "r"(v[4]), "r"(v[5]), "r"(v[6]), "r"(v[7]),
          "r"(v[8]), "r"(v[9]), "r"(v[10]), "r"(v[11]), "r"(v[12]), "r"(v[13]), "r"(v[14]), "r"(v[15])
        : "memory");
}
__device__ __forceinline__ void tc_wait_st() { asm volatile("tcgen05.wait::st.sync.aligned;" ::: "memory"); }

__device__ __forceinline__ uint64_t umma_desc_sw128(uint32_t smem_addr) {
    uint64_t d = 0;
    d |= static_cast<uint64_t>((smem_addr & 0x3FFFFu) >> 4);
    d |= static_cast<uint64_t>(1) << 16;
    d |= static_cast<uint64_t>(1024 >> 4) << 32;
    d |= static_cast<uint64_t>(1) << 46;
    d |= static_cast<uint64_t>(2) << 61;
    return d;
}
__host__ __device__ constexpr uint32_t umma_idesc_f16(uint32_t fmt, uint32_t M, uint32_t N) {
    return (1u << 4) | (fmt << 7) | (fmt << 10) | ((N >> 3) << 17) | ((M >> 4) << 24);
}

__device__ __forceinline__ int32_t f2ord(float f) {
    int32_t b = __float_as_int(f);
    return b >= 0 ? b : (b ^ 0x7FFFFFFF);
}
__device__ __forceinline__ float ord2f(int32_t o) {
    return __int_as_float(o >= 0 ? o : (o ^ 0x7FFFFFFF));
}
__device__ __forceinline__ int32_t ld_relaxed(const int32_t* p) {
    int32_t v;
    asm volatile("ld.relaxed.gpu.global.s32 %0, [%1];" : "=r"(v) : "l"(p) : "memory");
    return v;
}
__device__ __forceinline__ void st_relaxed(int32_t* p, int32_t v) {
    asm volatile("st.relaxed.gpu.global.s32 [%0], %1;" ::"l"(p), "r"(v) : "memory");
}

__device__ __forceinline__ float warp_dot128(const float4 a, const float* __restrict__ xrow, int lane) {
    const float4 b = reinterpret_cast<const float4*>(xrow)[lane];
    float s = a.x * b.x + a.y * b.y + a.z * b.z + a.w * b.w;
#pragma unroll
    for (int o = 16; o > 0; o >>= 1) s += __shfl_xor_sync(0xffffffffu, s, o);
    return s;
}

}
```

Baseline: 37950.

## Pair scan CTAs into 2-CTA clusters sharing multicast DB tiles across query halves

The flat scan kernel now launches in clusters of two CTAs. Each CTA handles one half of a doubled 512-query pass. Rank 0 issues TMA multicast loads of each database tile and its norms into both CTAs' shared memory, and signals the peer's barriers and tile index remotely. Empty-slot barriers now count arrivals from both CTAs' MMA commits. The goal is to halve global and L2 traffic per query and double queries per pass. The cost is cross-CTA synchronisation, half as many independent tile streams, and per-CTA pool and count layouts that the select and debug code must remap.

```diff
diff --git a/include/nafp.h b/include/nafp.h
--- a/include/nafp.h
+++ b/include/nafp.h
@@ -98,7 +98,7 @@
 
 int nafp_index_profile_scans(nafp_index* idx, int enable, double* total_ms, int64_t* n_scans);
 
-int nafp_index_debug_last_pass(nafp_index* idx, int32_t* flags256, float* thr256, int32_t* total256);
+int nafp_index_debug_last_pass(nafp_index* idx, int32_t* flags512, float* thr512, int32_t* total512);
 int nafp_index_debug_enable(nafp_index* idx, int32_t* cnt_out, int32_t* first_out, int32_t* grid_out);
 
 int nafp_seq_match(nafp_index* idx, const float* q_host, int64_t n_query_rows,
diff --git a/neural-audio-fp_b200/csrc/flat_search.cu b/neural-audio-fp_b200/csrc/flat_search.cu
--- a/neural-audio-fp_b200/csrc/flat_search.cu
+++ b/neural-audio-fp_b200/csrc/flat_search.cu
@@ -2,6 +2,7 @@
 #include <climits>
 #include <cstdlib>
 #include <cstring>
+#include <algorithm>
 #include <vector>
 
 #include "index.h"
@@ -78,11 +79,12 @@
 constexpr int PART_COLS = SCAN_TILE / EPI_PARTS;
 constexpr int SLOT_BYTES = SCAN_TILE * 128;
 constexpr int BOX_BYTES = TILE_ROWS * 128;
-constexpr int Q_KB_BYTES = NQ_MAX * 128;
+constexpr int Q_KB_BYTES = NQ_CTA * 128;
 constexpr int Q_BYTES_MAX = 2 * Q_KB_BYTES;
 constexpr int H_RING = 4;
 constexpr int WARM_TILES = 8;
-constexpr int SCAN_SMEM = Q_BYTES_MAX + RING_SLOTS * SLOT_BYTES + H_RING * SCAN_TILE * 4 + 2 * NQ_MAX * 4 + 256 + 1024;
+constexpr int SCAN_SMEM = Q_BYTES_MAX + RING_SLOTS * SLOT_BYTES + H_RING * SCAN_TILE * 4 + 3 * NQ_CTA * 4 + 256 + 1024;
+constexpr uint16_t PAIR_MASK = 0b11, RANK0_MASK = 0b01;
 constexpr int NEG_INF_ORD = static_cast<int>(0x807FFFFFu);
 static_assert(PART_COLS == 64, "epilogue reads two 32-column chunks per unit");
 
@@ -162,18 +164,21 @@
     uint8_t* b_s = smem + Q_BYTES_MAX;
     float* h_s = reinterpret_cast<float*>(b_s + RING_SLOTS * SLOT_BYTES);
     int* lmax_s = reinterpret_cast<int*>(h_s + H_RING * SCAN_TILE);
-    int* cnt_s = lmax_s + NQ_MAX;
-    ScanBars* bars = reinterpret_cast<ScanBars*>(cnt_s + NQ_MAX);
+    int* cnt_s = lmax_s + 2 * NQ_CTA;
+    ScanBars* bars = reinterpret_cast<ScanBars*>(cnt_s + NQ_CTA);
 
     const int warp = threadIdx.x >> 5;
     const int lane = threadIdx.x & 31;
     const int G = gridDim.x;
     const int cta = blockIdx.x;
+    const int rank = cta & 1, clu = cta >> 1, C = G >> 1;
+    const int qrow0 = rank * n_half * 128;
     const int warm_cap = ((tune >> 8) & 15) ? ((tune >> 8) & 15) : WARM_TILES;
-    const int warm = (tune & 2) ? 1 : max(1, min(warm_cap, n_tiles / G));
-
-    for (int i = threadIdx.x; i < NQ_MAX; i += blockDim.x) {
+    const int warm = (tune & 2) ? 1 : max(1, min(warm_cap, n_tiles / C));
+
+    for (int i = threadIdx.x; i < NQ_CTA; i += blockDim.x) {
         lmax_s[i] = INT_MIN;
+        lmax_s[NQ_CTA + i] = INT_MIN;
         cnt_s[i] = 0;
     }
     if (threadIdx.x == 0) {
@@ -181,7 +186,7 @@
         tma_prefetch_desc(&tmap_db);
         for (int s = 0; s < RING_SLOTS; ++s) {
             mbar_init(&bars->full[s], 1);
-            mbar_init(&bars->empty[s], 1);
+            mbar_init(&bars->empty[s], 2);
         }
         for (int a = 0; a < 2; ++a) {
             mbar_init(&bars->tfull[a], 1);
@@ -196,7 +201,7 @@
         tmem_relinquish();
     }
     tc_fence_before();
-    __syncthreads();
+    cluster_sync();
     tc_fence_after();
     const uint32_t tmem_base = __shfl_sync(0xffffffffu, bars->tmem_base, 0);
 
@@ -206,16 +211,23 @@
             mbar_arrive_expect_tx(&bars->qfull, 2u * q_rows * 128u);
             for (int kb = 0; kb < 2; ++kb)
                 for (int r0 = 0; r0 < q_rows; r0 += 32)
-                    tma_load_2d(q_s + kb * Q_KB_BYTES + r0 * 128, &tmap_q, &bars->qfull, kb * 64, r0);
-            int tile = cta;
+                    tma_load_2d(q_s + kb * Q_KB_BYTES + r0 * 128, &tmap_q, &bars->qfull, kb * 64, qrow0 + r0);
+        }
+        if (lane == 0 && rank == 0) {
+            const uint32_t peer_full0 = map_shared_rank(&bars->full[0], 1);
+            const uint32_t peer_tile_of0 = map_shared_rank(&bars->tile_of[0], 1);
+            int tile = clu;
             int revisit = -1;
-            int nxt = warm * G + atomicAdd(tile_counter, 1);
-            for (int i = 0;; ++i) {
+            int nxt = warm * C + atomicAdd(tile_counter, 1);
+            int i = 0;
+            for (;; ++i) {
                 const int kc0 = 2 * i;
                 const uint32_t ph = (kc0 / RING_SLOTS) & 1;
                 const int s0 = kc0 % RING_SLOTS;
                 mbar_wait_parked(&bars->empty[s0], ph ^ 1);
                 bars->tile_of[i & 7] = tile;
+                mbar_arrive_expect_tx_remote(peer_full0 + 8 * s0, (tile < 0 ? 0 : SLOT_BYTES + SCAN_TILE * 4) + 4);
+                st_async_remote(peer_tile_of0 + 4 * (i & 7), tile, peer_full0 + 8 * s0);
                 if (tile < 0) {
                     mbar_arrive(&bars->full[s0]);
                     break;
@@ -223,25 +235,31 @@
 #pragma unroll
                 for (int kb = 0; kb < 2; ++kb) {
                     const int s = s0 + kb;
-                    if (kb == 1) mbar_wait_parked(&bars->empty[s], ph ^ 1);
+                    if (kb == 1) {
+                        mbar_wait_parked(&bars->empty[s], ph ^ 1);
+                        mbar_arrive_expect_tx_remote(peer_full0 + 8 * s, SLOT_BYTES);
+                    }
                     mbar_arrive_expect_tx(&bars->full[s], SLOT_BYTES + (kb == 0 ? SCAN_TILE * 4 : 0));
                     if (kb == 0)
-                        bulk_load_1d(h_s + (i % H_RING) * SCAN_TILE, hn + static_cast<int64_t>(tile) * SCAN_TILE, SCAN_TILE * 4,
-                                     &bars->full[s]);
+                        bulk_load_1d_multicast(h_s + (i % H_RING) * SCAN_TILE, hn + static_cast<int64_t>(tile) * SCAN_TILE,
+                                               SCAN_TILE * 4, &bars->full[s], PAIR_MASK);
                     uint8_t* dst = b_s + s * SLOT_BYTES;
-                    tma_load_2d(dst, &tmap_db, &bars->full[s], kb * 64, tile * SCAN_TILE);
-                    tma_load_2d(dst + BOX_BYTES, &tmap_db, &bars->full[s], kb * 64, tile * SCAN_TILE + TILE_ROWS);
+                    tma_load_2d_multicast(dst, &tmap_db, &bars->full[s], kb * 64, tile * SCAN_TILE, PAIR_MASK);
+                    tma_load_2d_multicast(dst + BOX_BYTES, &tmap_db, &bars->full[s], kb * 64, tile * SCAN_TILE + TILE_ROWS,
+                                          PAIR_MASK);
                 }
                 if (i + 1 < warm) {
-                    tile = cta + (i + 1) * G;
+                    tile = clu + (i + 1) * C;
                 } else if (revisit < 0 && nxt < n_tiles) {
                     tile = nxt;
-                    nxt = warm * G + atomicAdd(tile_counter, 1);
+                    nxt = warm * C + atomicAdd(tile_counter, 1);
                 } else {
                     ++revisit;
-                    tile = revisit < warm ? cta + revisit * G : -1;
-                }
-            }
+                    tile = revisit < warm ? clu + revisit * C : -1;
+                }
+            }
+            for (int kc = 2 * i + 1; kc < 2 * i + RING_SLOTS; ++kc)
+                mbar_wait_parked(&bars->empty[kc % RING_SLOTS], ((kc / RING_SLOTS) & 1) ^ 1);
         }
         __syncwarp();
     } else if (warp == MMA_WARP) {
@@ -261,7 +279,7 @@
                 const bool last = hq == n_half - 1;
                 mbar_wait_parked(&bars->tempty[acc], aph ^ 1);
                 if (hq == 0) {
-                    mbar_wait_parked(&bars->full[s0], ph);
+                    mbar_wait_parked_cluster(&bars->full[s0], ph);
                     if (smem_ld_volatile(&bars->tile_of[i & 7]) < 0) {
                         if (leader) tc_commit(&bars->tfull[acc]);
                         __syncwarp();
@@ -278,16 +296,16 @@
                 if (leader) {
 #pragma unroll
                     for (int j = 0; j < 4; ++j) tc_mma_f16(d_tmem, a_kb0 + 2 * j, b_kb0 + 2 * j, idesc, j != 0 ? 1u : 0u);
-                    if (last) tc_commit(&bars->empty[s0]);
+                    if (last) tc_commit_multicast(&bars->empty[s0], RANK0_MASK);
                 }
                 if (hq == 0) {
-                    mbar_wait_parked(&bars->full[s1], ph);
+                    mbar_wait_parked_cluster(&bars->full[s1], ph);
                     tc_fence_after();
                 }
                 if (leader) {
 #pragma unroll
                     for (int j = 0; j < 4; ++j) tc_mma_f16(d_tmem, a_kb1 + 2 * j, b_kb1 + 2 * j, idesc, 1u);
-                    if (last) tc_commit(&bars->empty[s1]);
+                    if (last) tc_commit_multicast(&bars->empty[s1], RANK0_MASK);
                     tc_commit(&bars->tfull[acc]);
                 }
                 __syncwarp();
@@ -298,7 +316,10 @@
         const int qd = warp & 3;
         const int e = warp;
         const int part = e >> 2;
-        constexpr int QPW = NQ_MAX / EPI_WARPS;
+        constexpr int QPW = NQ_CTA / EPI_WARPS;
+        static_assert(2 * QPW == 32, "one lane per (query, column half) when maxima are published");
+        const int q_rows = n_half * 128;
+        int* lmax_part = lmax_s + (part >> 1) * NQ_CTA;
         const float NEG_INF = -INFINITY;
         int pub = INT_MIN;
         int thr_ord[2] = {NEG_INF_ORD, NEG_INF_ORD};
@@ -306,15 +327,15 @@
         bool active[2];
 #pragma unroll
         for (int hq = 0; hq < 2; ++hq) {
-            active[hq] = hq < n_half && (hq * 128 + qd * 32 + lane) < nq;
+            active[hq] = hq < n_half && qrow0 + (hq * 128 + qd * 32 + lane) < nq;
             t_exact[hq] = active[hq] ? NEG_INF : INFINITY;
             t_pre[hq] = t_exact[hq];
         }
-        uint64_t* my_pool = pool + static_cast<int64_t>(cta) * NQ_MAX * POOL_CAP;
+        uint64_t* my_pool = pool + static_cast<int64_t>(cta) * NQ_CTA * POOL_CAP;
         const uint32_t ns32 = static_cast<uint32_t>(n_search);
         auto load_thresholds = [&](int (&tg)[2]) {
 #pragma unroll
-            for (int hq = 0; hq < 2; ++hq) tg[hq] = active[hq] ? ld_relaxed(&Tg[hq * 128 + qd * 32 + lane]) : INT_MIN;
+            for (int hq = 0; hq < 2; ++hq) tg[hq] = active[hq] ? ld_relaxed(&Tg[qrow0 + hq * 128 + qd * 32 + lane]) : INT_MIN;
         };
         auto apply_thresholds = [&](const int (&tg)[2], int i) -> bool {
             bool valid = true;
@@ -323,7 +344,7 @@
                 if (active[hq]) {
                     if (tg[hq] > thr_ord[hq]) {
                         if (dbg_first && part == 0 && thr_ord[hq] == NEG_INF_ORD)
-                            dbg_first[cta * NQ_MAX + hq * 128 + qd * 32 + lane] = i;
+                            dbg_first[cta * NQ_MAX + qrow0 + hq * 128 + qd * 32 + lane] = i;
                         thr_ord[hq] = tg[hq];
                         const float t = ord2f(tg[hq]);
                         t_exact[hq] = t;
@@ -335,32 +356,32 @@
             return __all_sync(0xffffffffu, valid);
         };
         auto publish_maxima = [&]() {
-            const int q = e * QPW + lane;
-            if (lane < QPW && q < nq) {
-                const int m = smem_ld_volatile(&lmax_s[q]);
+            const int ql = e * QPW + (lane % QPW), half = lane / QPW;
+            if (ql < q_rows && qrow0 + ql < nq) {
+                const int m = smem_ld_volatile(&lmax_s[half * NQ_CTA + ql]);
                 if (m > pub) {
-                    st_relaxed(&Mx[q * G + cta], m);
+                    st_relaxed(&Mx[(qrow0 + ql) * G + 2 * clu + half], m);
                     pub = m;
                 }
             }
         };
-        const bool probe = dbg_first != nullptr && threadIdx.x == 0 && nq <= 248;
+        const bool probe = dbg_first != nullptr && threadIdx.x == 0 && nq <= NQ_MAX - 8;
         unsigned long long t_start = 0;
         if (probe) asm volatile("mov.u64 %0, %%globaltimer;" : "=l"(t_start));
         auto stamp = [&](int slot) {
             if (probe) {
                 unsigned long long t;
                 asm volatile("mov.u64 %0, %%globaltimer;" : "=l"(t));
-                dbg_first[cta * NQ_MAX + 248 + slot] = static_cast<int>(t - t_start);
+                dbg_first[cta * NQ_MAX + NQ_MAX - 8 + slot] = static_cast<int>(t - t_start);
             }
         };
         const uint32_t tlane = tmem_base + (static_cast<uint32_t>(qd * 32) << 16) + part * PART_COLS;
         uint32_t uc = 0;
 
         for (int w = 0; w < warm; ++w) {
-            const uint32_t row0 = static_cast<uint32_t>(cta + w * G) * SCAN_TILE + part * PART_COLS;
+            const uint32_t row0 = static_cast<uint32_t>(clu + w * C) * SCAN_TILE + part * PART_COLS;
             const float* h_part = h_s + (w % H_RING) * SCAN_TILE + part * PART_COLS;
-            bool edge = (static_cast<uint32_t>(cta + w * G) + 1u) * SCAN_TILE > ns32 || (tune & 4);
+            bool edge = (static_cast<uint32_t>(clu + w * C) + 1u) * SCAN_TILE > ns32 || (tune & 4);
             float hx = 0.f;
             for (int hq = 0; hq < n_half; ++hq, ++uc) {
                 const int acc = uc & 1;
@@ -397,7 +418,7 @@
                             if (j < nvalid) munit = fmaxf(munit, __uint_as_float(v[j]) - hc[j]);
                     }
                 }
-                if (hq == 0 ? active[0] : active[1]) smem_red_max(&lmax_s[hq * 128 + qd * 32 + lane], f2ord(munit));
+                if (hq == 0 ? active[0] : active[1]) smem_red_max(&lmax_part[hq * 128 + qd * 32 + lane], f2ord(munit));
                 tc_fence_before();
                 __syncwarp();
                 mbar_arrive_lane0(&bars->tempty[acc], lane);
@@ -462,10 +483,10 @@
                         const float te = hq == 0 ? t_exact[0] : t_exact[1];
                         const uint32_t rbase = row0 + c * 32;
                         if (!edge)
-                            scan_chunk_hits<false>(v, h_part + c * 32, te, 32, rbase, &cnt_s[q], &lmax_s[q], my_pool + q * POOL_CAP);
+                            scan_chunk_hits<false>(v, h_part + c * 32, te, 32, rbase, &cnt_s[q], &lmax_part[q], my_pool + q * POOL_CAP);
                         else
                             scan_chunk_hits<true>(v, h_part + c * 32, te, static_cast<int>(min(ns32 - min(ns32, rbase), 32u)), rbase,
-                                                  &cnt_s[q], &lmax_s[q], my_pool + q * POOL_CAP);
+                                                  &cnt_s[q], &lmax_part[q], my_pool + q * POOL_CAP);
                         __syncwarp();
                     }
                 }
@@ -487,11 +508,11 @@
         __syncwarp();
         asm volatile("bar.sync 1, %0;" ::"n"(EPI_WARPS * 32) : "memory");
         {
-            const int q = e * QPW + lane;
-            if (lane < QPW && q < nq) {
-                const int c = cnt_s[q];
-                cnt[cta * NQ_MAX + q] = min(c, POOL_CAP);
-                if (c > POOL_CAP) flags[q] = 1;
+            const int ql = e * QPW + lane;
+            if (lane < QPW && ql < q_rows && qrow0 + ql < nq) {
+                const int c = cnt_s[ql];
+                cnt[cta * NQ_CTA + ql] = min(c, POOL_CAP);
+                if (c > POOL_CAP) flags[qrow0 + ql] = 1;
             }
         }
         if (lane == 0) smem_atom_inc(&bars->done);
@@ -528,7 +549,7 @@
     }
 
     tc_fence_before();
-    __syncthreads();
+    cluster_sync();
     if (warp == MMA_WARP) tmem_dealloc(tmem_base, 512);
 }
 
@@ -561,6 +582,7 @@
 
 struct SelBatch {
     int np[SEL_SLOTS];
+    int h[SEL_SLOTS];
     int grid_alloc;
 };
 
@@ -580,8 +602,8 @@
     q32 += static_cast<int64_t>(slot) * NQ_MAX * D128;
     qn2 += slot * NQ_MAX;
     Tg += slot * NQ_MAX;
-    pool += static_cast<int64_t>(slot) * batch.grid_alloc * NQ_MAX * POOL_CAP;
-    cnt += static_cast<int64_t>(slot) * batch.grid_alloc * NQ_MAX;
+    pool += static_cast<int64_t>(slot) * batch.grid_alloc * NQ_CTA * POOL_CAP;
+    cnt += static_cast<int64_t>(slot) * batch.grid_alloc * NQ_CTA;
     flags += slot * NQ_MAX;
     gidx += slot * NQ_MAX;
     const int64_t g = gidx[q];
@@ -595,12 +617,14 @@
     if (threadIdx.x == 0) total_s = 0;
     __syncthreads();
     bool over = false;
-    for (int g = threadIdx.x; g < grid_scan; g += blockDim.x) {
-        const int c = cnt[g * NQ_MAX + q];
+    const int rank = q / batch.h[slot], ql = q - rank * batch.h[slot];
+    for (int pr = threadIdx.x; pr < grid_scan / 2; pr += blockDim.x) {
+        const int cta = 2 * pr + rank;
+        const int c = cnt[cta * NQ_CTA + ql];
         if (c > 0) {
             const int base = atomicAdd(&total_s, c);
             if (base + c <= SELECT_CAP) {
-                const uint64_t* src = pool + (static_cast<int64_t>(g) * NQ_MAX + q) * POOL_CAP;
+                const uint64_t* src = pool + (static_cast<int64_t>(cta) * NQ_CTA + ql) * POOL_CAP;
                 for (int i = 0; i < c; ++i) keys[base + i] = src[i];
             } else {
                 over = true;
@@ -868,19 +892,40 @@
     return NAFP_OK;
 }
 
+static cudaLaunchConfig_t scan_launch_config(int grid, cudaStream_t stream, cudaLaunchAttribute (&attr)[1]) {
+    attr[0].id = cudaLaunchAttributeClusterDimension;
+    attr[0].val.clusterDim.x = 2;
+    attr[0].val.clusterDim.y = 1;
+    attr[0].val.clusterDim.z = 1;
+    cudaLaunchConfig_t cfg = {};
+    cfg.gridDim = dim3(grid);
+    cfg.blockDim = dim3(SCAN_THREADS);
+    cfg.dynamicSmemBytes = SCAN_SMEM;
+    cfg.stream = stream;
+    cfg.attrs = attr;
+    cfg.numAttrs = 1;
+    return cfg;
+}
+
 static int ensure_scratch(nafp_index* idx) {
     if (idx->scratch_ready) return NAFP_OK;
     nafp_ctx* ctx = idx->ctx;
-    idx->grid = ctx->sm_count;
-    NAFP_REQUIRE(idx->grid <= 160, NAFP_ERR_UNSUPPORTED, "flat scan: %d SMs (reducer handles <= 160)", idx->grid);
+    NAFP_CUDA(cudaFuncSetAttribute(flat_scan_kernel, cudaFuncAttributeMaxDynamicSharedMemorySize, SCAN_SMEM));
+    cudaLaunchAttribute attr[1];
+    const cudaLaunchConfig_t cfg = scan_launch_config(2 * (ctx->sm_count / 2), ctx->stream, attr);
+    int clusters = 0;
+    NAFP_CUDA(cudaOccupancyMaxActiveClusters(&clusters, flat_scan_kernel, &cfg));
+    NAFP_REQUIRE(clusters >= 1, NAFP_ERR_UNSUPPORTED, "flat scan: no CTA pair of the scan kernel fits on this device");
+    idx->grid = 2 * clusters;
+    NAFP_REQUIRE(idx->grid <= 160, NAFP_ERR_UNSUPPORTED, "flat scan: %d CTAs (reducer handles <= 160)", idx->grid);
     const int G = idx->grid;
     NAFP_CUDA(cudaMalloc(&idx->qbf, NQ_MAX * D128 * sizeof(__nv_bfloat16)));
     NAFP_CUDA(cudaMalloc(&idx->q32, SEL_SLOTS * NQ_MAX * D128 * sizeof(float)));
     NAFP_CUDA(cudaMalloc(&idx->qn2, SEL_SLOTS * NQ_MAX * sizeof(float)));
     NAFP_CUDA(cudaMalloc(&idx->Mx, static_cast<size_t>(NQ_MAX) * G * sizeof(int32_t)));
     NAFP_CUDA(cudaMalloc(&idx->Tg, SEL_SLOTS * NQ_MAX * sizeof(int32_t)));
-    NAFP_CUDA(cudaMalloc(&idx->pool, SEL_SLOTS * static_cast<size_t>(G) * NQ_MAX * POOL_CAP * sizeof(uint64_t)));
-    NAFP_CUDA(cudaMalloc(&idx->cnt, SEL_SLOTS * static_cast<size_t>(G) * NQ_MAX * sizeof(int32_t)));
+    NAFP_CUDA(cudaMalloc(&idx->pool, SEL_SLOTS * static_cast<size_t>(G) * NQ_CTA * POOL_CAP * sizeof(uint64_t)));
+    NAFP_CUDA(cudaMalloc(&idx->cnt, SEL_SLOTS * static_cast<size_t>(G) * NQ_CTA * sizeof(int32_t)));
     NAFP_CUDA(cudaMalloc(&idx->flags, SEL_SLOTS * NQ_MAX * sizeof(int32_t)));
     NAFP_CUDA(cudaMalloc(&idx->gidx, SEL_SLOTS * NQ_MAX * sizeof(int64_t)));
     NAFP_CUDA(cudaMalloc(&idx->brute_part, static_cast<size_t>(BRUTE_SLOTS) * BRUTE_CHUNKS * MAX_K * sizeof(uint64_t)));
@@ -892,7 +937,6 @@
     const uint32_t box[2] = {64, 32};
     NAFP_TRY(make_tensor_map(&idx->tmap_q, CU_TENSOR_MAP_DATA_TYPE_BFLOAT16, 2, idx->qbf, dims, strides, box, nullptr,
                              CU_TENSOR_MAP_SWIZZLE_128B));
-    NAFP_CUDA(cudaFuncSetAttribute(flat_scan_kernel, cudaFuncAttributeMaxDynamicSharedMemorySize, SCAN_SMEM));
     idx->scratch_ready = true;
     return NAFP_OK;
 }
@@ -920,29 +964,32 @@
 static int scan_pass(nafp_index* idx, const float* q_dev, const int32_t* src_list, int src_off, int64_t p0, int np, int kg,
                      int grid_scan, int n_tiles, int64_t n_search, int slot) {
     nafp_ctx* ctx = idx->ctx;
-    const int n_half = np > 128 ? 2 : 1;
-    const int nq_pad = n_half * 128;
+    const int n_half = np > NQ_MAX / 2 ? 2 : 1;
+    const int nq_pad = 2 * n_half * 128;
     const int64_t G = idx->grid;
     float* q32 = idx->q32 + static_cast<int64_t>(slot) * NQ_MAX * D128;
     float* qn2 = idx->qn2 + slot * NQ_MAX;
     int32_t* Tg = idx->Tg + slot * NQ_MAX;
-    uint64_t* pool = idx->pool + static_cast<int64_t>(slot) * G * NQ_MAX * POOL_CAP;
-    int32_t* cnt = idx->cnt + static_cast<int64_t>(slot) * G * NQ_MAX;
+    uint64_t* pool = idx->pool + static_cast<int64_t>(slot) * G * NQ_CTA * POOL_CAP;
+    int32_t* cnt = idx->cnt + static_cast<int64_t>(slot) * G * NQ_CTA;
     int32_t* flags = idx->flags + slot * NQ_MAX;
     int64_t* gidx = idx->gidx + slot * NQ_MAX;
     flat_prep_kernel<<<(nq_pad * 32 + 255) / 256, 256, 0, ctx->stream>>>(q_dev, src_list, src_off, p0, np, nq_pad, grid_scan,
                                                                          idx->qbf, q32, qn2, idx->Mx, Tg, flags, gidx, idx->tile_counter);
     const bool prof = idx->profile && idx->prof_n < PROF_RING;
     if (prof) cudaEventRecord(idx->prof_ev[2 * idx->prof_n], ctx->stream);
-    flat_scan_kernel<<<grid_scan, SCAN_THREADS, SCAN_SMEM, ctx->stream>>>(idx->tmap_q, idx->tmap_db, idx->hn, idx->tile_counter, n_search,
-                                                                          n_tiles, np, n_half, kg, idx->Mx, Tg, pool, cnt, flags,
-                                                                          idx->dbg_first, scan_tune());
+    cudaLaunchAttribute attr[1];
+    const cudaLaunchConfig_t cfg = scan_launch_config(grid_scan, ctx->stream, attr);
+    NAFP_CUDA(cudaLaunchKernelEx(&cfg, flat_scan_kernel, idx->tmap_q, idx->tmap_db, static_cast<const float*>(idx->hn),
+                                 idx->tile_counter, n_search, n_tiles, np, n_half, kg, idx->Mx, Tg, pool, cnt, flags,
+                                 idx->dbg_first, scan_tune()));
     if (prof) {
         cudaEventRecord(idx->prof_ev[2 * idx->prof_n + 1], ctx->stream);
         idx->prof_n++;
     }
     ctx->launches += 2;
     idx->last_slot = slot;
+    idx->last_h = n_half * 128;
     return NAFP_OK;
 }
 
@@ -969,7 +1016,7 @@
     const int64_t n_search = (idx->search_rows >= 0 && idx->search_rows < idx->n) ? idx->search_rows : idx->n;
     const int n_tiles = static_cast<int>((n_search + SCAN_TILE - 1) / SCAN_TILE);
     const int kg = k + 28;
-    const int grid_scan = n_tiles < idx->grid ? (n_tiles > 0 ? n_tiles : 1) : idx->grid;
+    const int grid_scan = 2 * std::max(1, std::min(n_tiles, idx->grid / 2));
     const bool brute = (n_search < 8192) || (kg > grid_scan) || (k > 64);
     idx->host_rows += nq;
     if (brute) return brute_rounds(idx, q_dev, nullptr, 0, nq, k, n_search, D_dev, I_dev);
@@ -991,6 +1038,7 @@
     for (int64_t p0 = 0; p0 < nq; p0 += NQ_MAX) {
         const int np = static_cast<int>(nq - p0 < NQ_MAX ? nq - p0 : NQ_MAX);
         NAFP_TRY(scan_pass(idx, q_dev, nullptr, 0, p0, np, kg, grid_scan, n_tiles, n_search, slot));
+        batch.h[slot] = idx->last_h;
         batch.np[slot++] = np;
         idx->host_passes++;
         if (slot == SEL_SLOTS || p0 + NQ_MAX >= nq) {
@@ -1008,6 +1056,7 @@
         for (int off = 0; off < h[0]; off += NQ_MAX) {
             const int np = h[0] - off < NQ_MAX ? h[0] - off : NQ_MAX;
             NAFP_TRY(scan_pass(idx, q_dev, list1, off, 0, np, kg_retry, grid_scan, n_tiles, n_search, slot));
+            batch.h[slot] = idx->last_h;
             batch.np[slot++] = np;
             idx->host_passes++;
             if (slot == SEL_SLOTS || off + NQ_MAX >= h[0]) {
@@ -1185,6 +1234,16 @@
     return NAFP_OK;
 }
 
+static int last_pass_counts(nafp_index* idx, std::vector<int32_t>& by_row) {
+    const size_t n_cta = static_cast<size_t>(idx->grid) * NQ_CTA;
+    std::vector<int32_t> cnt(n_cta);
+    NAFP_CUDA(cudaMemcpy(cnt.data(), idx->cnt + idx->last_slot * n_cta, n_cta * 4, cudaMemcpyDeviceToHost));
+    by_row.assign(static_cast<size_t>(idx->grid) * NQ_MAX, 0);
+    for (int g = 0; g < idx->grid; ++g)
+        for (int ql = 0; ql < idx->last_h; ++ql) by_row[static_cast<size_t>(g) * NQ_MAX + (g & 1) * idx->last_h + ql] = cnt[g * NQ_CTA + ql];
+    return NAFP_OK;
+}
+
 int nafp_index_debug_enable(nafp_index* idx, int32_t* cnt_out, int32_t* first_out, int32_t* grid_out) {
     NAFP_REQUIRE(idx && idx->scratch_ready, NAFP_ERR_STATE, "debug: search once first");
     nafp_ctx* ctx = idx->ctx;
@@ -1195,7 +1254,11 @@
         NAFP_CUDA(cudaMemset(idx->dbg_first, 0xFF, n * 4));
     }
     if (grid_out) *grid_out = idx->grid;
-    if (cnt_out) NAFP_CUDA(cudaMemcpy(cnt_out, idx->cnt + static_cast<size_t>(idx->last_slot) * n, n * 4, cudaMemcpyDeviceToHost));
+    if (cnt_out) {
+        std::vector<int32_t> by_row;
+        NAFP_TRY(last_pass_counts(idx, by_row));
+        memcpy(cnt_out, by_row.data(), n * 4);
+    }
     if (first_out) {
         NAFP_CUDA(cudaMemcpy(first_out, idx->dbg_first, n * 4, cudaMemcpyDeviceToHost));
         NAFP_CUDA(cudaMemset(idx->dbg_first, 0xFF, n * 4));
@@ -1203,21 +1266,21 @@
     return NAFP_OK;
 }
 
-int nafp_index_debug_last_pass(nafp_index* idx, int32_t* flags256, float* thr256, int32_t* total256) {
-    NAFP_REQUIRE(idx && idx->scratch_ready && flags256 && thr256 && total256, NAFP_ERR_INVALID, "debug: bad arguments");
+int nafp_index_debug_last_pass(nafp_index* idx, int32_t* flags_out, float* thr_out, int32_t* total_out) {
+    NAFP_REQUIRE(idx && idx->scratch_ready && flags_out && thr_out && total_out, NAFP_ERR_INVALID, "debug: bad arguments");
     nafp_ctx* ctx = idx->ctx;
     NAFP_CUDA(cudaStreamSynchronize(ctx->stream));
-    std::vector<int32_t> tg(NQ_MAX), cnt(static_cast<size_t>(idx->grid) * NQ_MAX);
-    NAFP_CUDA(cudaMemcpy(flags256, idx->flags + idx->last_slot * NQ_MAX, NQ_MAX * 4, cudaMemcpyDeviceToHost));
+    std::vector<int32_t> tg(NQ_MAX), cnt;
+    NAFP_CUDA(cudaMemcpy(flags_out, idx->flags + idx->last_slot * NQ_MAX, NQ_MAX * 4, cudaMemcpyDeviceToHost));
     NAFP_CUDA(cudaMemcpy(tg.data(), idx->Tg + idx->last_slot * NQ_MAX, NQ_MAX * 4, cudaMemcpyDeviceToHost));
-    NAFP_CUDA(cudaMemcpy(cnt.data(), idx->cnt + static_cast<size_t>(idx->last_slot) * cnt.size(), cnt.size() * 4, cudaMemcpyDeviceToHost));
+    NAFP_TRY(last_pass_counts(idx, cnt));
     for (int q = 0; q < NQ_MAX; ++q) {
         int32_t o = tg[q];
         uint32_t b = static_cast<uint32_t>(o >= 0 ? o : (o ^ 0x7FFFFFFF));
-        memcpy(&thr256[q], &b, 4);
+        memcpy(&thr_out[q], &b, 4);
         int64_t t = 0;
         for (int g = 0; g < idx->grid; ++g) t += cnt[static_cast<size_t>(g) * NQ_MAX + q];
-        total256[q] = static_cast<int32_t>(t);
+        total_out[q] = static_cast<int32_t>(t);
     }
     return NAFP_OK;
 }
diff --git a/neural-audio-fp_b200/csrc/index.h b/neural-audio-fp_b200/csrc/index.h
--- a/neural-audio-fp_b200/csrc/index.h
+++ b/neural-audio-fp_b200/csrc/index.h
@@ -7,7 +7,8 @@
 namespace nafp {
 
 constexpr int D128 = 128;
-constexpr int NQ_MAX = 256;
+constexpr int NQ_MAX = 512;
+constexpr int NQ_CTA = 256;
 constexpr int TILE_ROWS = 128;
 constexpr int SCAN_TILE = 256;
 constexpr int POOL_CAP = 128;
@@ -39,6 +40,7 @@
     bool tmap_db_valid = false;
 
     int last_slot = 0;
+    int last_h = 0;
     bool scratch_ready = false;
     int grid = 0;
     __nv_bfloat16* qbf = nullptr;
diff --git a/neural-audio-fp_b200/csrc/ptx.cuh b/neural-audio-fp_b200/csrc/ptx.cuh
--- a/neural-audio-fp_b200/csrc/ptx.cuh
+++ b/neural-audio-fp_b200/csrc/ptx.cuh
@@ -62,6 +62,39 @@
         if (++spins > (1u << 24)) __trap();
     }
 }
+__device__ __forceinline__ void mbar_wait_parked_cluster(uint64_t* bar, uint32_t parity) {
+    uint32_t spins = 0;
+    for (;;) {
+        uint32_t ok;
+        asm volatile(
+            "{\n\t.reg .pred P;\n\t"
+            "mbarrier.try_wait.parity.acquire.cluster.shared::cta.b64 P, [%1], %2, %3;\n\t"
+            "selp.u32 %0, 1, 0, P;\n\t}\n"
+            : "=r"(ok)
+            : "r"(smem_u32(bar)), "r"(parity), "r"(2000u)
+            : "memory");
+        if (ok) return;
+        if (++spins > (1u << 24)) __trap();
+    }
+}
+
+__device__ __forceinline__ void cluster_sync() {
+    asm volatile("barrier.cluster.arrive.release.aligned;\n\tbarrier.cluster.wait.acquire.aligned;" ::: "memory");
+}
+__device__ __forceinline__ uint32_t map_shared_rank(const void* p, uint32_t rank) {
+    uint32_t r;
+    asm volatile("mapa.shared::cluster.u32 %0, %1, %2;" : "=r"(r) : "r"(smem_u32(p)), "r"(rank));
+    return r;
+}
+__device__ __forceinline__ void mbar_arrive_expect_tx_remote(uint32_t bar_cluster, uint32_t bytes) {
+    asm volatile("mbarrier.arrive.expect_tx.relaxed.cluster.shared::cluster.b64 _, [%0], %1;" ::"r"(bar_cluster), "r"(bytes)
+                 : "memory");
+}
+__device__ __forceinline__ void st_async_remote(uint32_t dst_cluster, int32_t v, uint32_t bar_cluster) {
+    asm volatile("st.async.shared::cluster.mbarrier::complete_tx::bytes.b32 [%0], %1, [%2];" ::"r"(dst_cluster), "r"(v),
+                 "r"(bar_cluster)
+                 : "memory");
+}
 
 __device__ __forceinline__ void tma_prefetch_desc(const void* tmap) {
     asm volatile("prefetch.tensormap [%0];" ::"l"(reinterpret_cast<uint64_t>(tmap)) : "memory");
@@ -70,6 +103,13 @@
     asm volatile(
         "cp.async.bulk.tensor.2d.shared::cluster.global.mbarrier::complete_tx::bytes [%0], [%1, {%3, %4}], [%2];"
         ::"r"(smem_u32(smem_dst)), "l"(reinterpret_cast<uint64_t>(tmap)), "r"(smem_u32(bar)), "r"(c0), "r"(c1)
+        : "memory");
+}
+__device__ __forceinline__ void tma_load_2d_multicast(void* smem_dst, const void* tmap, uint64_t* bar, int32_t c0, int32_t c1,
+                                                      uint16_t cta_mask) {
+    asm volatile(
+        "cp.async.bulk.tensor.2d.shared::cluster.global.mbarrier::complete_tx::bytes.multicast::cluster [%0], [%1, {%3, %4}], [%2], %5;"
+        ::"r"(smem_u32(smem_dst)), "l"(reinterpret_cast<uint64_t>(tmap)), "r"(smem_u32(bar)), "r"(c0), "r"(c1), "h"(cta_mask)
         : "memory");
 }
 __device__ __forceinline__ void tma_load_3d(void* smem_dst, const void* tmap, uint64_t* bar, int32_t c0, int32_t c1, int32_t c2) {
@@ -137,6 +177,12 @@
                  "l"(reinterpret_cast<uint64_t>(gsrc)), "r"(bytes), "r"(smem_u32(bar))
                  : "memory");
 }
+__device__ __forceinline__ void bulk_load_1d_multicast(void* smem_dst, const void* gsrc, uint32_t bytes, uint64_t* bar,
+                                                       uint16_t cta_mask) {
+    asm volatile("cp.async.bulk.shared::cluster.global.mbarrier::complete_tx::bytes.multicast::cluster [%0], [%1], %2, [%3], %4;"
+                 ::"r"(smem_u32(smem_dst)), "l"(reinterpret_cast<uint64_t>(gsrc)), "r"(bytes), "r"(smem_u32(bar)), "h"(cta_mask)
+                 : "memory");
+}
 __device__ __forceinline__ void fence_proxy_async_smem() {
     asm volatile("fence.proxy.async.shared::cta;" ::: "memory");
 }
@@ -164,6 +210,11 @@
 }
 __device__ __forceinline__ void tc_commit(uint64_t* bar) {
     asm volatile("tcgen05.commit.cta_group::1.mbarrier::arrive::one.shared::cluster.b64 [%0];" ::"r"(smem_u32(bar)) : "memory");
+}
+__device__ __forceinline__ void tc_commit_multicast(uint64_t* bar, uint16_t cta_mask) {
+    asm volatile("tcgen05.commit.cta_group::1.mbarrier::arrive::one.shared::cluster.multicast::cluster.b64 [%0], %1;"
+                 ::"r"(smem_u32(bar)), "h"(cta_mask)
+                 : "memory");
 }
 
 __device__ __forceinline__ void tmem_ld_32x32(uint32_t taddr, uint32_t (&v)[32]) {
```

Result: faster. 43460, median of 6 (+14.5%).
